# uwoseis/zephyr

Measured on AMD Instinct MI355X. Metric: wavefields/sec (freq x source solves/s) on 1024^2 grid, higher is better.
Workload: dtype f64

## Files before the change

include/helm.h:

```cpp
#ifndef HELM_H
#define HELM_H

#include <stddef.h>

#ifdef __cplusplus
extern "C" {
#endif

typedef struct helm_op helm_op;

enum { HELM_MINIZEPHYR = 0, HELM_EURUS = 1, HELM_3D = 2  };

enum {
    HELM_BICGSTAB = 0,
    HELM_CGNR = 1,
    HELM_AUTO = 2,
    HELM_MG = 3,
    HELM_DIRECT = 4
};

enum {
    HELM_OK = 0,
    HELM_ERR_ARG = -1,
    HELM_ERR_DEVICE = -2,
    HELM_ERR_STATE = -3,
    HELM_ERR_UNSUPPORTED = -4,
    HELM_ERR_PML = -5
};

enum { HELM_RHS_NODE_MAJOR = 1, HELM_OUT_NODE_MAJOR = 2, HELM_NODE_MAJOR = 3 };

typedef struct helm_solve_opts {
    int method;
    double rtol;
    int maxit;
    int check_every;
    int batch;
    int flags;
} helm_solve_opts;

typedef struct helm_solve_info {
    int iterations;
    int status;
    int restarts;
    int method;
    double relres;
} helm_solve_info;

int helm_device_count(void);
const char *helm_version(void);

helm_op *helm_create(int device, int variant, int nz, int nx, double dx, double dz,
                     int nPML, const int *freeSurf);
helm_op *helm_create3d(int device, int nz, int ny, int nx, double dx, double dy, double dz, int nPML);
void helm_destroy(helm_op *op);
const char *helm_last_error(const helm_op *op);

int helm_set_stream(helm_op *op, void *hip_stream);

int helm_set_model(helm_op *op, const double *c, const double *rho,
                   const double *theta, const double *eps, const double *delta);

int helm_assemble(helm_op *op, double freq_re, double freq_im, double tau, double ky, double cPML);

int helm_num_blocks(const helm_op *op);
long long helm_num_points(const helm_op *op);

int helm_get_diagonals(helm_op *op, double *out);

int helm_apply(helm_op *op, int block, int adjoint, const double *X, double *Y, int nrhs);
int helm_apply_device(helm_op *op, int block, int adjoint, const void *dX, void *dY, int nrhs);

int helm_solve(helm_op *op, const double *RHS, double *U, int nrhs, long long rows,
               double premul_re, double premul_im,
               const helm_solve_opts *opts, helm_solve_info *info);
int helm_solve_device(helm_op *op, const void *dRHS, void *dU, int nrhs, long long rows,
                      double premul_re, double premul_im,
                      const helm_solve_opts *opts, helm_solve_info *info);

int helm_solve_coo(helm_op *op, const long long *row, const int *col, const double *val, long long nnz, double *U, int nrhs,
                   long long rows, double premul_re, double premul_im, const helm_solve_opts *opts, helm_solve_info *info);
void *helm_host_alloc(size_t bytes);
void helm_host_free(void *p, size_t bytes);

int helm_prefactor(helm_op *op);
int helm_prefactor_n(helm_op *op, int nrhs);
int helm_prefactor_many(helm_op **ops, int n);
int helm_set_tolerance_hint(helm_op *op, double rtol);

int helm_reserve(helm_op *op, int nrhs, long long rows, int concurrent);

typedef struct helm_timing {
    double solve_ms;
    double apply_ms;
    long long apply_launches;
    double apply_bytes;
    double factor_ms;
    double gemm_ms;
    long long gemm_launches;
    double gemm_flops;
    double gemm_big_ms;
    long long gemm_big_launches;
    double gemm_big_flops;
    double gemm_bytes;
    double gemm_sol_ms;
} helm_timing;
int helm_last_timing(const helm_op *op, helm_timing *out);
int helm_set_profiling(helm_op *op, int on);

int helm_imaging_accumulate_device(helm_op *op, const void *dUF, const void *dUB, int nsrc,
                                   const void *dScaler, void *dG);

int helm_rhs_from_coo_device(helm_op *op, const void *d_row, const void *d_col, const void *d_val, long long nnz,
                             void *dR, int nrhs, long long rows);
int helm_rhs_from_coo_device_layout(helm_op *op, const void *d_row, const void *d_col, const void *d_val, long long nnz,
                                    void *dR, int nrhs, long long rows, int flags);

int helm_set_rhs_support(helm_op *op, const void *d_bits, long long rows, int nrhs);
int helm_rhs_support_from_coo(helm_op *op, const void *d_row, const void *d_col, long long nnz, void *d_bits, long long rows, int nrhs);
int helm_sample_device(helm_op *op, const void *dU, int nsrc, long long ld, const void *d_rowptr, const void *d_col,
                       const void *d_val, int nrec, void *d_out);
int helm_sample_accumulate_device(helm_op *op, const void *dU, int nsrc, long long ld, const void *d_rowptr, const void *d_col,
                                  const void *d_val, int nrec, double alpha_re, double alpha_im, double beta_re, double beta_im, void *d_out);
int helm_axpby_device(helm_op *op, double alpha_re, double alpha_im, const void *dX, double beta_re, double beta_im, void *dY, long long n);

int helm_pool_spares(int device, int spare);
int helm_trim(void);
int helm_host_trim(void);
int helm_debug_ws_slots(int device, long long bytes);
int helm_debug_plan_cache(int device);
int helm_debug_ws_selftest(int ndev, int concurrent, long long bytes);
int helm_debug_alloc_stats(int reset, long long *slow_calls, double *worst_ms);

int helm_warm(int device);
typedef struct helm_runtime_stats {
    long long dev_allocs;  double dev_alloc_bytes;  double dev_alloc_ms;
    long long host_allocs; double host_alloc_bytes; double host_alloc_ms;
    long long events_created, streams_created;
    long long first_launches; double first_launch_ms;
    long long kernels_registered, kernels_resolved; double warm_ms;
    long long dev_frees; double dev_free_ms;
    long long sync_calls; double sync_ms;
    long long slow_syncs; double worst_sync_ms;
} helm_runtime_stats;
int helm_debug_runtime_stats(int reset, helm_runtime_stats *out);
int helm_debug_stall_watch(int start, double *worst_gap_ms, long long *gaps_over_5ms);

typedef struct helm_tuning {
    int    nd_leaf;
    double nd_ws_gb;
    int    nd_sparse_rhs;
    int    nd_stable;
    double nd_stable_thr;
    double nd_stable_safety;
    int    nd_fused_leaf;
    int    nd_fused_leaf_min;
    int    nd_gjstep;
    int    nd_gjstep_min;
    int    nd_overlap;
    int    nd_xcd_map;
    int    nd_plans;
    int    nd_direct_out;
    int    nd_many;
    int    nd_leaf_idle;
    int    auto_direct;
    int    auto_mg3;
    int    prof_ext;
    int    ws_slots;
    int    pf_prio;
    int    mg3_keep;
    int    mg3_keep_levels;
    int    mg3_galerkin;
    int    mg3_depth_model;
    int    mg3_bt_f32;
    int    mg3_otf;
    int    mg3_f32;
    double mg3_omega;
    double sync_spin_ms;
    int    sync_sleep_us;
} helm_tuning;
int helm_get_tuning(helm_tuning *out);
int helm_set_tuning(const helm_tuning *t);

int helm_direct_plan(int nz, int nx, int leaf, int *out, int cap);
int helm_direct_plan_front(int nz, int nx, int leaf, int node, long long *cells, int cap);
int helm_debug_zgemm(int device, int M, int N, int K, const double *alpha, const double *A, const double *B,
                     const double *beta, double *C, int batch);
int helm_debug_inverse(int device, int n, double *A, int batch);
int helm_debug_zgemm_bench(int device, int M, int N, int K, int batch, int variant, int reps, double *ms_out);
#define HELM_ZG_TABLE 1
#define HELM_ZG_MASKS 2
#define HELM_ZG_TM64  4
int helm_debug_zgemm_choice(int M, int N, int K, int batch, int nf_div, int force_tile, int force_slab, int have_handle, int mode, int report[5]);
typedef struct helm_zgemm_ex {
    int device, M, N, K, batch;
    int lda, ldb, ldc;
    long long sa, sb, sc;
    double alpha[2], beta[2];
    const double *A; long long a_len;
    double *B; long long b_len;
    double *C; long long c_len;
    int force_tile, force_slab;
    int xcd_map;
    int ntc;
    int zr0, zr1, zc0, zc1, sk0, sk1;
    int tm64, c_is_b;
    const int *tabB, *tabCi, *tabCo; long long tab_len;
    int tab_stride, offB, offCi, offCo;
    int ldx; long long arena_rows;
    const double *Bx, *Bx2, *Cix;
    double *Cox, *Cox2;
    int k2, cj_out; double oscale[2];
    int *act;
    int report[5];
} helm_zgemm_ex;
int helm_debug_zgemm_ex(helm_zgemm_ex *p);
int helm_debug_inverse_bench(int device, int n, const double *A, int reps, int recurse_n, double *ms_out);

int helm_mg3_axis(int n, int npml, double h, double cpml, double om_re, double om_im, int level, double *x, int *lay, double *lap,
                  int *pc, double *pw, int *n_next, int *rf, double *rw);

int helm_regrid_axis(int n_in, double h_in, int n_out, double h_out, int *start, double *taps, int cap);
typedef struct helm_regrid helm_regrid;
helm_regrid *helm_regrid_create(int device, int nz_a, int nx_a, double dz_a, double dx_a, int nz_b, int nx_b, double dz_b, double dx_b,
                                double zorig, double xorig);
void helm_regrid_destroy(helm_regrid *plan);
int helm_regrid_apply_device(helm_regrid *plan, helm_op *op, int k, const void *dIn, long long in_fstride, long long in_estride, void *dOut,
                             long long out_fstride, long long out_estride, double gain_re, double gain_im, double beta, const void *dMul);
int helm_regrid_apply(helm_regrid *plan, int k, const double *in, long long in_fstride, long long in_estride, double *out, long long out_fstride,
                      long long out_estride, double gain_re, double gain_im, double beta, const double *mul);

#ifdef __cplusplus
}
#endif
#endif
```

zephyr_amd/_lib.py:

```python
import ctypes
import os
import numpy as np

_HERE = os.path.dirname(os.path.abspath(__file__))
LIB_PATH = os.path.join(_HERE, 'libhelm.so')

HELM_MINIZEPHYR, HELM_EURUS, HELM_3D = 0, 1, 2
HELM_BICGSTAB, HELM_CGNR, HELM_AUTO, HELM_MG, HELM_DIRECT = 0, 1, 2, 3, 4
HELM_RHS_NODE_MAJOR, HELM_OUT_NODE_MAJOR, HELM_NODE_MAJOR = 1, 2, 3
METHODS = {'bicgstab': HELM_BICGSTAB, 'cgnr': HELM_CGNR, 'auto': HELM_AUTO, 'mg': HELM_MG, 'direct': HELM_DIRECT}

ERRORS = {-1: 'HELM_ERR_ARG', -2: 'HELM_ERR_DEVICE', -3: 'HELM_ERR_STATE', -4: 'HELM_ERR_UNSUPPORTED', -5: 'HELM_ERR_PML'}


class HelmError(RuntimeError):
    def __init__(self, code, text):
        self.code = code
        RuntimeError.__init__(self, '%s: %s' % (ERRORS.get(code, code), text))


class SolveOpts(ctypes.Structure):
    _fields_ = [('method', ctypes.c_int), ('rtol', ctypes.c_double), ('maxit', ctypes.c_int),
                ('check_every', ctypes.c_int), ('batch', ctypes.c_int), ('flags', ctypes.c_int)]


class SolveInfo(ctypes.Structure):
    _fields_ = [('iterations', ctypes.c_int), ('status', ctypes.c_int), ('restarts', ctypes.c_int),
                ('method', ctypes.c_int), ('relres', ctypes.c_double)]


class Timing(ctypes.Structure):
    _fields_ = [('solve_ms', ctypes.c_double), ('apply_ms', ctypes.c_double),
                ('apply_launches', ctypes.c_longlong), ('apply_bytes', ctypes.c_double),
                ('factor_ms', ctypes.c_double), ('gemm_ms', ctypes.c_double),
                ('gemm_launches', ctypes.c_longlong), ('gemm_flops', ctypes.c_double),
                ('gemm_big_ms', ctypes.c_double), ('gemm_big_launches', ctypes.c_longlong), ('gemm_big_flops', ctypes.c_double),
                ('gemm_bytes', ctypes.c_double), ('gemm_sol_ms', ctypes.c_double)]


class Tuning(ctypes.Structure):
    _fields_ = [('nd_leaf', ctypes.c_int), ('nd_ws_gb', ctypes.c_double), ('nd_sparse_rhs', ctypes.c_int), ('nd_stable', ctypes.c_int),
                ('nd_stable_thr', ctypes.c_double), ('nd_stable_safety', ctypes.c_double), ('nd_fused_leaf', ctypes.c_int),
                ('nd_fused_leaf_min', ctypes.c_int), ('nd_gjstep', ctypes.c_int), ('nd_gjstep_min', ctypes.c_int), ('nd_overlap', ctypes.c_int),
                ('nd_xcd_map', ctypes.c_int), ('nd_plans', ctypes.c_int), ('nd_direct_out', ctypes.c_int), ('nd_many', ctypes.c_int), ('nd_leaf_idle', ctypes.c_int), ('auto_direct', ctypes.c_int),
                ('auto_mg3', ctypes.c_int), ('prof_ext', ctypes.c_int), ('ws_slots', ctypes.c_int), ('pf_prio', ctypes.c_int),
                ('mg3_keep', ctypes.c_int), ('mg3_keep_levels', ctypes.c_int), ('mg3_galerkin', ctypes.c_int), ('mg3_depth_model', ctypes.c_int),
                ('mg3_bt_f32', ctypes.c_int), ('mg3_otf', ctypes.c_int), ('mg3_f32', ctypes.c_int), ('mg3_omega', ctypes.c_double), ('sync_spin_ms', ctypes.c_double), ('sync_sleep_us', ctypes.c_int)]


class RuntimeStats(ctypes.Structure):
    _fields_ = [('dev_allocs', ctypes.c_longlong), ('dev_alloc_bytes', ctypes.c_double), ('dev_alloc_ms', ctypes.c_double),
                ('host_allocs', ctypes.c_longlong), ('host_alloc_bytes', ctypes.c_double), ('host_alloc_ms', ctypes.c_double),
                ('events_created', ctypes.c_longlong), ('streams_created', ctypes.c_longlong),
                ('first_launches', ctypes.c_longlong), ('first_launch_ms', ctypes.c_double),
                ('kernels_registered', ctypes.c_longlong), ('kernels_resolved', ctypes.c_longlong), ('warm_ms', ctypes.c_double),
                ('dev_frees', ctypes.c_longlong), ('dev_free_ms', ctypes.c_double),
                ('sync_calls', ctypes.c_longlong), ('sync_ms', ctypes.c_double), ('slow_syncs', ctypes.c_longlong), ('worst_sync_ms', ctypes.c_double)]


class ZgemmEx(ctypes.Structure):
    _fields_ = [('device', ctypes.c_int), ('M', ctypes.c_int), ('N', ctypes.c_int), ('K', ctypes.c_int), ('batch', ctypes.c_int),
                ('lda', ctypes.c_int), ('ldb', ctypes.c_int), ('ldc', ctypes.c_int),
                ('sa', ctypes.c_longlong), ('sb', ctypes.c_longlong), ('sc', ctypes.c_longlong),
                ('alpha', ctypes.c_double * 2), ('beta', ctypes.c_double * 2),
                ('A', ctypes.c_void_p), ('a_len', ctypes.c_longlong), ('B', ctypes.c_void_p), ('b_len', ctypes.c_longlong),
                ('C', ctypes.c_void_p), ('c_len', ctypes.c_longlong),
                ('force_tile', ctypes.c_int), ('force_slab', ctypes.c_int), ('xcd_map', ctypes.c_int), ('ntc', ctypes.c_int),
                ('zr0', ctypes.c_int), ('zr1', ctypes.c_int), ('zc0', ctypes.c_int), ('zc1', ctypes.c_int), ('sk0', ctypes.c_int), ('sk1', ctypes.c_int),
                ('tm64', ctypes.c_int), ('c_is_b', ctypes.c_int),
                ('tabB', ctypes.c_void_p), ('tabCi', ctypes.c_void_p), ('tabCo', ctypes.c_void_p), ('tab_len', ctypes.c_longlong),
                ('tab_stride', ctypes.c_int), ('offB', ctypes.c_int), ('offCi', ctypes.c_int), ('offCo', ctypes.c_int),
                ('ldx', ctypes.c_int), ('arena_rows', ctypes.c_longlong),
                ('Bx', ctypes.c_void_p), ('Bx2', ctypes.c_void_p), ('Cix', ctypes.c_void_p), ('Cox', ctypes.c_void_p), ('Cox2', ctypes.c_void_p),
                ('k2', ctypes.c_int), ('cj_out', ctypes.c_int), ('oscale', ctypes.c_double * 2),
                ('act', ctypes.c_void_p), ('report', ctypes.c_int * 5)]


_c_dp = ctypes.POINTER(ctypes.c_double)
_SIGNATURES = {
    'helm_device_count': (ctypes.c_int, []),
    'helm_version': (ctypes.c_char_p, []),
    'helm_create': (ctypes.c_void_p, [ctypes.c_int, ctypes.c_int, ctypes.c_int, ctypes.c_int, ctypes.c_double,
                                      ctypes.c_double, ctypes.c_int, ctypes.POINTER(ctypes.c_int)]),
    'helm_create3d': (ctypes.c_void_p, [ctypes.c_int, ctypes.c_int, ctypes.c_int, ctypes.c_int, ctypes.c_double,
                                        ctypes.c_double, ctypes.c_double, ctypes.c_int]),
    'helm_destroy': (None, [ctypes.c_void_p]),
    'helm_last_error': (ctypes.c_char_p, [ctypes.c_void_p]),
    'helm_set_stream': (ctypes.c_int, [ctypes.c_void_p, ctypes.c_void_p]),
    'helm_set_model': (ctypes.c_int, [ctypes.c_void_p, ctypes.c_void_p, ctypes.c_void_p, ctypes.c_void_p,
                                      ctypes.c_void_p, ctypes.c_void_p]),
    'helm_assemble': (ctypes.c_int, [ctypes.c_void_p, ctypes.c_double, ctypes.c_double, ctypes.c_double,
                                     ctypes.c_double, ctypes.c_double]),
    'helm_num_blocks': (ctypes.c_int, [ctypes.c_void_p]),
    'helm_num_points': (ctypes.c_longlong, [ctypes.c_void_p]),
    'helm_get_diagonals': (ctypes.c_int, [ctypes.c_void_p, ctypes.c_void_p]),
    'helm_apply': (ctypes.c_int, [ctypes.c_void_p, ctypes.c_int, ctypes.c_int, ctypes.c_void_p, ctypes.c_void_p, ctypes.c_int]),
    'helm_apply_device': (ctypes.c_int, [ctypes.c_void_p, ctypes.c_int, ctypes.c_int, ctypes.c_void_p, ctypes.c_void_p, ctypes.c_int]),
    'helm_solve': (ctypes.c_int, [ctypes.c_void_p, ctypes.c_void_p, ctypes.c_void_p, ctypes.c_int, ctypes.c_longlong,
                                  ctypes.c_double, ctypes.c_double, ctypes.POINTER(SolveOpts), ctypes.POINTER(SolveInfo)]),
    'helm_solve_device': (ctypes.c_int, [ctypes.c_void_p, ctypes.c_void_p, ctypes.c_void_p, ctypes.c_int, ctypes.c_longlong,
                                         ctypes.c_double, ctypes.c_double, ctypes.POINTER(SolveOpts), ctypes.POINTER(SolveInfo)]),
    'helm_solve_coo': (ctypes.c_int, [ctypes.c_void_p, ctypes.c_void_p, ctypes.c_void_p, ctypes.c_void_p, ctypes.c_longlong, ctypes.c_void_p, ctypes.c_int,
                                      ctypes.c_longlong, ctypes.c_double, ctypes.c_double, ctypes.POINTER(SolveOpts), ctypes.POINTER(SolveInfo)]),
    'helm_host_alloc': (ctypes.c_void_p, [ctypes.c_size_t]),
    'helm_host_free': (None, [ctypes.c_void_p, ctypes.c_size_t]),
    'helm_rhs_from_coo_device_layout': (ctypes.c_int, [ctypes.c_void_p, ctypes.c_void_p, ctypes.c_void_p, ctypes.c_void_p, ctypes.c_longlong,
                                                       ctypes.c_void_p, ctypes.c_int, ctypes.c_longlong, ctypes.c_int]),
    'helm_prefactor': (ctypes.c_int, [ctypes.c_void_p]),
    'helm_prefactor_n': (ctypes.c_int, [ctypes.c_void_p, ctypes.c_int]),
    'helm_prefactor_many': (ctypes.c_int, [ctypes.POINTER(ctypes.c_void_p), ctypes.c_int]),
    'helm_reserve': (ctypes.c_int, [ctypes.c_void_p, ctypes.c_int, ctypes.c_longlong, ctypes.c_int]),
    'helm_set_tolerance_hint': (ctypes.c_int, [ctypes.c_void_p, ctypes.c_double]),
    'helm_last_timing': (ctypes.c_int, [ctypes.c_void_p, ctypes.POINTER(Timing)]),
    'helm_set_profiling': (ctypes.c_int, [ctypes.c_void_p, ctypes.c_int]),
    'helm_imaging_accumulate_device': (ctypes.c_int, [ctypes.c_void_p, ctypes.c_void_p, ctypes.c_void_p, ctypes.c_int,
                                                      ctypes.c_void_p, ctypes.c_void_p]),
    'helm_get_tuning': (ctypes.c_int, [ctypes.POINTER(Tuning)]),
    'helm_set_tuning': (ctypes.c_int, [ctypes.POINTER(Tuning)]),
    'helm_pool_spares': (ctypes.c_int, [ctypes.c_int, ctypes.c_int]),
    'helm_trim': (ctypes.c_int, []),
    'helm_host_trim': (ctypes.c_int, []),
    'helm_debug_ws_slots': (ctypes.c_int, [ctypes.c_int, ctypes.c_longlong]),
    'helm_debug_plan_cache': (ctypes.c_int, [ctypes.c_int]),
    'helm_debug_ws_selftest': (ctypes.c_int, [ctypes.c_int, ctypes.c_int, ctypes.c_longlong]),
    'helm_debug_alloc_stats': (ctypes.c_int, [ctypes.c_int, ctypes.POINTER(ctypes.c_longlong), ctypes.POINTER(ctypes.c_double)]),
    'helm_warm': (ctypes.c_int, [ctypes.c_int]),
    'helm_debug_runtime_stats': (ctypes.c_int, [ctypes.c_int, ctypes.POINTER(RuntimeStats)]),
    'helm_debug_stall_watch': (ctypes.c_int, [ctypes.c_int, ctypes.POINTER(ctypes.c_double), ctypes.POINTER(ctypes.c_longlong)]),
    'helm_rhs_from_coo_device': (ctypes.c_int, [ctypes.c_void_p, ctypes.c_void_p, ctypes.c_void_p, ctypes.c_void_p, ctypes.c_longlong,
                                                ctypes.c_void_p, ctypes.c_int, ctypes.c_longlong]),
    'helm_sample_device': (ctypes.c_int, [ctypes.c_void_p, ctypes.c_void_p, ctypes.c_int, ctypes.c_longlong, ctypes.c_void_p, ctypes.c_void_p,
                                          ctypes.c_void_p, ctypes.c_int, ctypes.c_void_p]),
    'helm_sample_accumulate_device': (ctypes.c_int, [ctypes.c_void_p, ctypes.c_void_p, ctypes.c_int, ctypes.c_longlong, ctypes.c_void_p, ctypes.c_void_p,
                                                     ctypes.c_void_p, ctypes.c_int, ctypes.c_double, ctypes.c_double, ctypes.c_double, ctypes.c_double,
                                                     ctypes.c_void_p]),
    'helm_axpby_device': (ctypes.c_int, [ctypes.c_void_p, ctypes.c_double, ctypes.c_double, ctypes.c_void_p, ctypes.c_double, ctypes.c_double,
                                         ctypes.c_void_p, ctypes.c_longlong]),
    'helm_direct_plan': (ctypes.c_int, [ctypes.c_int, ctypes.c_int, ctypes.c_int, ctypes.c_void_p, ctypes.c_int]),
    'helm_direct_plan_front': (ctypes.c_int, [ctypes.c_int, ctypes.c_int, ctypes.c_int, ctypes.c_int, ctypes.c_void_p, ctypes.c_int]),
    'helm_mg3_axis': (ctypes.c_int, [ctypes.c_int, ctypes.c_int, ctypes.c_double, ctypes.c_double, ctypes.c_double, ctypes.c_double, ctypes.c_int,
                                     ctypes.c_void_p, ctypes.c_void_p, ctypes.c_void_p, ctypes.c_void_p, ctypes.c_void_p, ctypes.c_void_p, ctypes.c_void_p,
                                     ctypes.c_void_p]),
    'helm_debug_zgemm': (ctypes.c_int, [ctypes.c_int, ctypes.c_int, ctypes.c_int, ctypes.c_int, ctypes.c_void_p, ctypes.c_void_p,
                                        ctypes.c_void_p, ctypes.c_void_p, ctypes.c_void_p, ctypes.c_int]),
    'helm_debug_zgemm_choice': (ctypes.c_int, [ctypes.c_int] * 9 + [ctypes.POINTER(ctypes.c_int)]),
    'helm_debug_zgemm_ex': (ctypes.c_int, [ctypes.POINTER(ZgemmEx)]),
    'helm_debug_inverse': (ctypes.c_int, [ctypes.c_int, ctypes.c_int, ctypes.c_void_p, ctypes.c_int]),
    'helm_debug_zgemm_bench': (ctypes.c_int, [ctypes.c_int, ctypes.c_int, ctypes.c_int, ctypes.c_int, ctypes.c_int, ctypes.c_int, ctypes.c_int,
                                              ctypes.POINTER(ctypes.c_double)]),
    'helm_set_rhs_support': (ctypes.c_int, [ctypes.c_void_p, ctypes.c_void_p, ctypes.c_longlong, ctypes.c_int]),
    'helm_rhs_support_from_coo': (ctypes.c_int, [ctypes.c_void_p, ctypes.c_void_p, ctypes.c_void_p, ctypes.c_longlong, ctypes.c_void_p, ctypes.c_longlong, ctypes.c_int]),
    'helm_regrid_axis': (ctypes.c_int, [ctypes.c_int, ctypes.c_double, ctypes.c_int, ctypes.c_double, ctypes.c_void_p, ctypes.c_void_p, ctypes.c_int]),
    'helm_regrid_create': (ctypes.c_void_p, [ctypes.c_int, ctypes.c_int, ctypes.c_int, ctypes.c_double, ctypes.c_double, ctypes.c_int, ctypes.c_int,
                                             ctypes.c_double, ctypes.c_double, ctypes.c_double, ctypes.c_double]),
    'helm_regrid_destroy': (None, [ctypes.c_void_p]),
    'helm_regrid_apply_device': (ctypes.c_int, [ctypes.c_void_p, ctypes.c_void_p, ctypes.c_int, ctypes.c_void_p, ctypes.c_longlong, ctypes.c_longlong,
                                                ctypes.c_void_p, ctypes.c_longlong, ctypes.c_longlong, ctypes.c_double, ctypes.c_double, ctypes.c_double,
                                                ctypes.c_void_p]),
    'helm_regrid_apply': (ctypes.c_int, [ctypes.c_void_p, ctypes.c_int, ctypes.c_void_p, ctypes.c_longlong, ctypes.c_longlong, ctypes.c_void_p,
                                         ctypes.c_longlong, ctypes.c_longlong, ctypes.c_double, ctypes.c_double, ctypes.c_double, ctypes.c_void_p]),
    'helm_debug_inverse_bench': (ctypes.c_int, [ctypes.c_int, ctypes.c_int, ctypes.c_void_p, ctypes.c_int, ctypes.c_int, ctypes.POINTER(ctypes.c_double)]),
}

_lib = None


def exported_symbols():
    return sorted(_SIGNATURES)


def load():
    global _lib
    if _lib is None:
        if os.environ.get('HELM_NO_TORCH_PRELOAD', '0') != '1':
            try:
                import torch
            except Exception:
                pass
        if not os.path.exists(LIB_PATH):
            raise ImportError('libhelm.so not found at %s: run `python -c "import __graft_entry__ as g; g.build()"` '
                              '(hipcc --offload-arch=gfx950).  There is no CPU fallback.' % LIB_PATH)
        lib = ctypes.CDLL(LIB_PATH)
        for name, (res, args) in _SIGNATURES.items():
            fn = getattr(lib, name)
            fn.restype = res
            fn.argtypes = args
        _lib = lib
    return _lib


def tuning():
    t = Tuning()
    check(load().helm_get_tuning(ctypes.byref(t)))
    return t


def set_tuning(t=None):
    check(load().helm_set_tuning(ctypes.byref(t) if t is not None else None))


def runtime_stats(reset=False):
    st = RuntimeStats()
    check(load().helm_debug_runtime_stats(1 if reset else 0, ctypes.byref(st)))
    return {k: getattr(st, k) for k, _ in RuntimeStats._fields_}


def last_error(handle=None):
    msg = load().helm_last_error(handle)
    return msg.decode() if msg else ''


def check(rc, handle=None):
    if rc < 0:
        raise HelmError(rc, last_error(handle))
    return rc


def require_gpu():
    n = load().helm_device_count()
    if n <= 0:
        raise HelmError(-2, 'no HIP device visible (%s); libhelm has no CPU path' % last_error(None))
    return n


class _PinnedBlock(object):

    def __init__(self, nbytes):
        self.nbytes = int(nbytes)
        self.ptr = load().helm_host_alloc(self.nbytes)
        if not self.ptr:
            raise MemoryError('helm_host_alloc(%d) failed' % self.nbytes)
        self.__array_interface__ = {'shape': (self.nbytes,), 'typestr': '|u1', 'data': (self.ptr, False), 'version': 3}

    def __del__(self):
        try:
            if self.ptr:
                load().helm_host_free(self.ptr, self.nbytes)
                self.ptr = None
        except Exception:
            pass


def pinned_empty(shape, dtype=np.complex128):
    n = int(np.prod(shape)) * np.dtype(dtype).itemsize
    if n == 0:
        return np.empty(shape, dtype=dtype)
    try:
        block = _PinnedBlock(n)
    except Exception:
        return np.empty(shape, dtype=dtype)
    return np.asarray(block).view(dtype).reshape(shape)


def pinned_reserve(shape, count, dtype=np.complex128):
    held = [pinned_empty(shape, dtype) for _ in range(int(count))]
    n = len(held)
    del held
    return n


def to_device(arr, dev, dtype=None):
    import torch
    a = np.ascontiguousarray(arr, dtype=dtype)
    if a.nbytes < (64 << 10):
        return torch.from_numpy(a).to(dev)
    host = pinned_empty(a.shape, a.dtype)
    host[...] = a
    return torch.from_numpy(host).to(dev)


_TORCH_NP = {'torch.complex128': np.complex128, 'torch.complex64': np.complex64, 'torch.float64': np.float64, 'torch.float32': np.float32,
             'torch.int64': np.int64, 'torch.int32': np.int32, 'torch.uint8': np.uint8}


def from_device(t):
    import torch
    t = t.contiguous()
    if t.numel() * t.element_size() < (64 << 10):
        return t.cpu().numpy()
    host = pinned_empty(tuple(t.shape), _TORCH_NP[str(t.dtype)])
    torch.from_numpy(host).copy_(t)
    return np.array(host)


def from_device_pinned(t):
    import torch
    t = t.contiguous()
    if t.numel() * t.element_size() < (64 << 10):
        return t.cpu().numpy()
    host = pinned_empty(tuple(t.shape), _TORCH_NP[str(t.dtype)])
    torch.from_numpy(host).copy_(t)
    return host


def wait_torch_stream(dev, spin_ms=None):
    import time
    import torch
    st = torch.cuda.current_stream(dev)
    budget = (tuning().sync_spin_ms if spin_ms is None else spin_ms) * 1e-3
    t0 = time.perf_counter()
    while budget > 0 and not st.query():
        if time.perf_counter() - t0 > budget:
            break
    st.synchronize()


def ptr(arr):
    return arr.ctypes.data_as(ctypes.c_void_p) if arr is not None else None


def c128(arr):
    return np.ascontiguousarray(arr, dtype=np.complex128)


def f64(arr):
    return np.ascontiguousarray(arr, dtype=np.float64)
```

zephyr_amd/csrc/direct.hpp:

```cpp
#pragma once
#include "helm_internal.hpp"
#include <memory>

struct NdDev {
    int z0, z1, x0, x1;
    int cut, pos;
    int dof;
    int s, m;
    int ntop, nbot, nleft, nright, xlo;
    int kid[2];
    int smax, mmax;
    long long foff;
    long long finv_off, f12_off;
    long long voff;
    long long roff;
};

struct NdGroup {
    int first = 0, cnt = 0, level = 0;
    bool leaf = false;
    int smax = 0, mmax = 0;
    long long foff = 0, voff = 0;
    long long roff = 0;
    long long finv = 0, g21 = 0, f12 = 0;
};

struct NdPlan {
    int nz = 0, nx = 0, leaf = 8, nlevels = 0, dof = 1;
    std::vector<NdDev> nodes;
    std::vector<NdGroup> groups;
    long long fac_elems = 0, fregion = 0, vregion = 0, work_elems = 0, total_rows = 0;
};

struct NdPlanDev {
    NdPlan plan;
    int device = 0;
    NdDev *d_nodes = nullptr;
    int4 *d_tab = nullptr;
    int *d_cellnode = nullptr;
    ~NdPlanDev();
};

struct NdStable {
    int node = -1;
    size_t group = 0;
    int smax = 0, mmax = 0;
    cplx *lu = nullptr;
    cplx *f21 = nullptr;
    int *piv = nullptr;
    cplx *vs = nullptr; size_t vs_elems = 0;
};

#define ND_NF_MAX 4
struct NdPlanesSet { const cplx *p[ND_NF_MAX]; };
struct NdFacShared {
    int device = 0;
    cplx *d_fac = nullptr; size_t fac_bytes = 0;
    double *d_est = nullptr; size_t est_elems = 0;
    ~NdFacShared();
};
struct NdFactor {
    std::shared_ptr<NdPlanDev> pd;
    int nf = 1, kf = 0;
    std::shared_ptr<NdFacShared> shared;
    cplx *d_fac = nullptr;
    int block = 0;
    double flops = 0;
    std::vector<NdStable> stable;
    double *d_est = nullptr; size_t est_elems = 0;
    int act_nct = 0;
    unsigned char *d_qmask = nullptr; size_t qmask_elems = 0;
    int *d_act = nullptr; size_t act_elems = 0;
    int *d_leafflag = nullptr; size_t leafflag_elems = 0;
    struct FlagSlot *flag_slot = nullptr; double flag_thr = 0;
};

inline cplx *nd_fac_at(const NdFactor *f, long long off, long long slot) { return f->d_fac + (long long)f->nf * off + (long long)f->kf * slot; }
inline long long nd_fac_stride(const NdFactor *f, long long slot) { return (long long)f->nf * slot; }

__host__ __device__ inline int nd_local(const NdDev &n, int nz, int nx, int z, int x, int comp = 0) {
    (void)nz; (void)nx;
    const int d = n.dof;
    if (n.cut < 0) { if (z >= n.z0 && z < n.z1 && x >= n.x0 && x < n.x1) return ((z - n.z0) * (n.x1 - n.x0) + (x - n.x0)) * d + comp; }
    else if (n.cut == 0) { if (z == n.pos && x >= n.x0 && x < n.x1) return (x - n.x0) * d + comp; }
    else { if (x == n.pos && z >= n.z0 && z < n.z1) return (z - n.z0) * d + comp; }
    const int wrow = n.ntop ? n.ntop : n.nbot;
    if (n.ntop && z == n.z0 - 1 && x >= n.xlo && x < n.xlo + wrow) return n.s + (x - n.xlo) * d + comp;
    if (n.nbot && z == n.z1 && x >= n.xlo && x < n.xlo + wrow) return n.s + (n.ntop + (x - n.xlo)) * d + comp;
    if (n.nleft && x == n.x0 - 1 && z >= n.z0 && z < n.z1) return n.s + (n.ntop + n.nbot + (z - n.z0)) * d + comp;
    if (n.nright && x == n.x1 && z >= n.z0 && z < n.z1) return n.s + (n.ntop + n.nbot + n.nleft + (z - n.z0)) * d + comp;
    return -1;
}

__host__ __device__ inline void nd_cell(const NdDev &n, int a, int &z, int &x, int &comp) {
    const int d = n.dof;
    if (a < n.s) {
        comp = a % d; a /= d;
        if (n.cut < 0) { const int w = n.x1 - n.x0; z = n.z0 + a / w; x = n.x0 + a % w; }
        else if (n.cut == 0) { z = n.pos; x = n.x0 + a; }
        else { z = n.z0 + a; x = n.pos; }
        return;
    }
    a -= n.s;
    comp = a % d; a /= d;
    if (a < n.ntop) { z = n.z0 - 1; x = n.xlo + a; return; }
    a -= n.ntop;
    if (a < n.nbot) { z = n.z1; x = n.xlo + a; return; }
    a -= n.nbot;
    if (a < n.nleft) { z = n.z0 + a; x = n.x0 - 1; return; }
    a -= n.nleft;
    z = n.z0 + a; x = n.x1;
}
__host__ __device__ inline void nd_cell(const NdDev &n, int a, int &z, int &x) { int comp; nd_cell(n, a, z, x, comp); }

__host__ __device__ inline int nd_pos(const NdDev &n, int a) { return a < n.s ? a : n.smax + (a - n.s); }

int nd_build_plan(NdPlan &P, int nz, int nx, int leaf, int dof = 1);
long long nd_factor_ws_elems(const NdPlan &P);
int nd_get_plan(helm_op *op, int leaf, int dof, std::shared_ptr<NdPlanDev> *out);
int nd_get_plan_dims(helm_op *op, int nz, int nx, int leaf, int dof, std::shared_ptr<NdPlanDev> *out);
int nd_factor(helm_op *op, int block, NdFactor *f, cplx *ws, const cplx *planes = nullptr);
int nd_factor_enqueue(helm_op *op, int block, NdFactor *f, cplx *ws, const cplx *planes = nullptr);
int nd_factor_enqueue_many(helm_op *op, int nf, helm_op *const *ops, NdFactor *const *fs, cplx *ws);
void nd_free(NdFactor *f);
long long nd_solve_ws_elems(const NdPlan &P, int nrhs);
int nd_solve(helm_op *op, NdFactor *f, const cplx *Xin, cplx *Xout, int nrhs, cplx *ws, int conj_out = 0);
int nd_axpy_one(helm_op *op, cplx *y, const cplx *x, long long n, int conj = 0);
struct NdDirectOut { cplx *U = nullptr; cplx oscale = {1.0, 0.0}; };
int nd_solve_nm(helm_op *op, NdFactor *f, const cplx *Qt, cplx *Xt, int nrhs, cplx *arenaV, const NdDirectOut *dout = nullptr);
int nd_factor_solve_nm(helm_op *op, int block, NdFactor *f, cplx *ws_factor, const cplx *planes, const cplx *Qt, cplx *Xt, int nrhs, cplx *arenaV,
                       hipStream_t side, float *factor_ms, const NdDirectOut *dout = nullptr);
int nd_recover_x(helm_op *op, const cplx *U, cplx *Xt, long long elems, cplx oscale);
int nd_prep_transpose_norm(helm_op *op, const cplx *rhs, long long rhs_ld, long long row_off, cplx premul, const cplx *sub, cplx *Qt, long long N, int nrhs,
                           double *part, int nblk_cap, int *nblk_out);
const unsigned char *nd_rhs_mask(helm_op *op, NdFactor *f);
struct NdResidExtra {
    int qnorm = 0;
    cplx *Uout = nullptr; int ldu = 0;
    cplx oscale = {1.0, 0.0};
    const unsigned char *qmask = nullptr;
    int xin_is_u = 0;
};
int nd_resid_nm(helm_op *op, const cplx *planes, const cplx *Xin, int ldin, cplx *Q, int ldq, const int *qmap, int ncol, int store, cplx *Rout,
                double *part, int nblk_cap, int *nblk_out, const NdResidExtra *ex = nullptr);
int nd_transpose(helm_op *op, const cplx *in, long long rows, long long cols, cplx *out);
int nd_scatter_add_cols(helm_op *op, cplx *Xt, int ldq, const int *d_cols, int k, const cplx *Dp, long long N);
int nd_pack_cols(helm_op *op, const cplx *Qt, int ldq, const int *d_cols, int k, cplx *Rp, long long N);
int nd_transpose_out(helm_op *op, const cplx *Xt, long long N, int nrhs, cplx *U, int conj);

int nd_dense_gemm(helm_op *op, int M, int N, int K, cplx alpha, const cplx *A, int lda, const cplx *B, int ldb, cplx beta, cplx *C, int ldc);
int nd_dense_gemm_batched(helm_op *op, int M, int N, int K, cplx alpha, const cplx *A, int lda, long long sa, const cplx *B, int ldb, long long sb,
                          cplx beta, cplx *C, int ldc, long long sc, int batch);
int nd_dense_inverse(helm_op *op, cplx *M, int n, cplx *W);
```

zephyr_amd/csrc/nd_factor.hip:

```cpp
#include "nd_internal.hpp"
#include <map>
#include <mutex>
#include <cstring>

namespace {

__device__ __forceinline__ long long mf_off(long long off, long long slot, int nf, int kf) { return (long long)nf * off + (long long)kf * slot; }
__device__ __forceinline__ cplx *front_entry(const NdDev &n, cplx *arenaF, cplx *fac, int r, int c, int nf = 1, int kf = 0, int fac_private = 0) {
    const int nmax = n.smax + n.mmax;
    if (r < n.smax) {
        return fac + (fac_private ? n.finv_off : mf_off(n.finv_off, (long long)n.smax * nmax, nf, kf)) + (long long)r * nmax + c;
    }
    return arenaF + mf_off(n.foff, (long long)n.mmax * nmax, nf, kf) + (long long)(r - n.smax) * nmax + c;
}

__global__ __launch_bounds__(256) void k_nd_assemble(const NdDev *nodes, int first, cplx *arenaF, cplx *fac, const cplx *planes, int nz, int nx) {
    const NdDev n = nodes[first + blockIdx.y];
    const long long N = (long long)nz * nx;
    const int tot = n.s + n.m;
    for (int a = blockIdx.x * blockDim.x + threadIdx.x; a < n.smax; a += gridDim.x * blockDim.x)
        if (a >= n.s) *front_entry(n, arenaF, fac, a, a) = cmake(1.0, 0.0);
    for (int a = blockIdx.x * blockDim.x + threadIdx.x; a < tot; a += gridDim.x * blockDim.x) {
        int z, x, ca;
        nd_cell(n, a, z, x, ca);
        const int ra = nd_pos(n, a);
        const int cb0 = n.dof > 2 ? max(ca - 1, 0) : 0, cb1 = n.dof > 2 ? min(ca + 1, n.dof - 1) : n.dof - 1;
        for (int cb = cb0; cb <= cb1; ++cb) {
            const cplx *pl = n.dof > 2 ? planes + (long long)(cb - ca + 1) * 9 * N * n.dof + (long long)ca * N
                                       : planes + (long long)(n.dof == 2 ? 2 * ca + cb : 0) * 9 * N;
            const long long pstride = n.dof > 2 ? N * n.dof : N;
            #pragma unroll
            for (int k = 0; k < 9; ++k) {
                const int z2 = z + k / 3 - 1, x2 = x + k % 3 - 1;
                if (z2 < 0 || z2 >= nz || x2 < 0 || x2 >= nx) continue;
                const int b = nd_local(n, nz, nx, z2, x2, cb);
                if (b < 0 || (a >= n.s && b >= n.s)) continue;
                *front_entry(n, arenaF, fac, ra, nd_pos(n, b)) = pl[(long long)k * pstride + (long long)z * nx + x];
            }
        }
    }
}

__global__ __launch_bounds__(256) void k_nd_extend_add(const NdDev *nodes, int first, int slot, cplx *arenaF, cplx *fac, int nz, int nx, int chunk) {
    extern __shared__ int map[];
    const NdDev p = nodes[first + blockIdx.y];
    if (p.kid[slot] < 0) return;
    const NdDev c = nodes[p.kid[slot]];
    const long long total = (long long)c.m * c.m;
    if ((long long)blockIdx.x * chunk >= total) return;
    for (int a = threadIdx.x; a < c.m; a += blockDim.x) {
        int z, x, comp;
        nd_cell(c, c.s + a, z, x, comp);
        map[a] = nd_pos(p, nd_local(p, nz, nx, z, x, comp));
    }
    __syncthreads();
    const cplx *Sc = arenaF + c.foff + c.smax;
    const int ldc = c.smax + c.mmax;
    for (long long e0 = (long long)blockIdx.x * chunk; e0 < total; e0 += (long long)gridDim.x * chunk) {
        const long long e1 = e0 + chunk < total ? e0 + chunk : total;
        for (long long e = e0 + threadIdx.x; e < e1; e += blockDim.x) {
            const int a = (int)(e / c.m), b2 = (int)(e - (long long)a * c.m);
            cplx *dst = front_entry(p, arenaF, fac, map[a], map[b2]);
            *dst = cadd(*dst, Sc[(long long)a * ldc + b2]);
        }
    }
}

template <bool OVR>
__global__ __launch_bounds__(256) void k_nd_build_front(const NdDev *nodes, int first, cplx *arenaF, cplx *fac, NdPlanesSet pset, int nz, int nx, int rb,
                                                        int skip22, NdDev ovr, int nf, int kfix) {
    constexpr int use_ovr = OVR ? 1 : 0;
    extern __shared__ int2 finfo[];
    const int kf = kfix >= 0 ? kfix : (int)(blockIdx.y % nf);
    const cplx *planes = pset.p[kf];
    NdDev n;
    if (OVR) n = ovr; else n = nodes[first + (kfix >= 0 ? blockIdx.y : blockIdx.y / nf)];
    const int nmax = n.smax + n.mmax;
    const int r0 = blockIdx.x * rb;
    if (r0 >= nmax) return;
    const bool h0 = n.kid[0] >= 0, h1 = n.kid[1] >= 0;
    NdDev c0 = NdDev(), c1 = NdDev();
    if (h0) c0 = nodes[n.kid[0]];
    if (h1) c1 = nodes[n.kid[1]];
    const int tid = threadIdx.x;
    for (int r = tid; r < nmax; r += 256) {
        int a = -1;
        if (r < n.s) a = r;
        else if (r >= n.smax && r - n.smax < n.m) a = n.s + r - n.smax;
        int2 e = make_int2(-1, 0);
        if (a >= 0) {
            int z, x, comp;
            nd_cell(n, a, z, x, comp);
            int k0 = 0, k1 = 0;
            if (h0) { const int la = nd_local(c0, nz, nx, z, x, comp); if (la >= c0.s) k0 = la - c0.s + 1; }
            if (h1) { const int la = nd_local(c1, nz, nx, z, x, comp); if (la >= c1.s) k1 = la - c1.s + 1; }
            if (n.dof > 2) { e.x = z | (x << 12) | (comp << 24); e.y = k0 | (k1 << 16); }
            else { e.x = z | (x << 16); e.y = k0 | (k1 << 14) | (comp << 28); }
        }
        finfo[r] = e;
    }
    __syncthreads();
    const long long N = (long long)nz * nx;
    const int ld0 = c0.smax + c0.mmax, ld1 = c1.smax + c1.mmax;
    const cplx *S0 = h0 ? arenaF + mf_off(c0.foff, (long long)c0.mmax * ld0, nf, kf) + c0.smax : nullptr;
    const cplx *S1 = h1 ? arenaF + mf_off(c1.foff, (long long)c1.mmax * ld1, nf, kf) + c1.smax : nullptr;
    const int r1 = r0 + rb < nmax ? r0 + rb : nmax;
    const int tx = tid & 63, ty = tid >> 6;
    const bool colmode = n.dof > 2;
    auto value = [&](int r, int c, const int2 ia, const int2 ib) -> cplx {
        cplx v = cmake(0.0, 0.0);
        if (ia.x < 0 || ib.x < 0) { if (r == c && r < n.smax) v = cmake(1.0, 0.0); return v; }
        const int za = colmode ? (ia.x & 0xfff) : (ia.x & 0xffff), xa = colmode ? ((ia.x >> 12) & 0xfff) : (ia.x >> 16);
        const int ca = colmode ? ((ia.x >> 24) & 0x7f) : ((ia.y >> 28) & 1);
        const int a0 = (colmode ? (ia.y & 0xffff) : (ia.y & 0x3fff)) - 1, a1 = (colmode ? ((ia.y >> 16) & 0xffff) : ((ia.y >> 14) & 0x3fff)) - 1;
        if (r < n.smax || c < n.smax) {
            const int zb = colmode ? (ib.x & 0xfff) : (ib.x & 0xffff), xb = colmode ? ((ib.x >> 12) & 0xfff) : (ib.x >> 16);
            const int dz = zb - za, dx = xb - xa;
            if (dz >= -1 && dz <= 1 && dx >= -1 && dx <= 1) {
                if (colmode) {
                    const int dc = ((ib.x >> 24) & 0x7f) - ca;
                    if (dc >= -1 && dc <= 1) v = planes[((long long)(dc + 1) * 9 + (dz + 1) * 3 + dx + 1) * N * n.dof + (long long)ca * N + (long long)za * nx + xa];
                } else {
                    const int blk = n.dof == 2 ? 2 * ca + ((ib.y >> 28) & 1) : 0;
                    v = planes[((long long)blk * 9 + (dz + 1) * 3 + dx + 1) * N + (long long)za * nx + xa];
                }
            }
        }
        const int b0 = (colmode ? (ib.y & 0xffff) : (ib.y & 0x3fff)) - 1, b1 = (colmode ? ((ib.y >> 16) & 0xffff) : ((ib.y >> 14) & 0x3fff)) - 1;
        if (a0 >= 0 && b0 >= 0) v = cadd(v, S0[(long long)a0 * ld0 + b0]);
        if (a1 >= 0 && b1 >= 0) v = cadd(v, S1[(long long)a1 * ld1 + b1]);
        return v;
    };
    for (int r = r0 + ty; r < r1; r += 4) {
        const int2 ia = finfo[r];
        const int cend = (skip22 && r >= n.smax) ? n.smax : nmax;
        for (int c = tx; c < cend; c += 64) *front_entry(n, arenaF, fac, r, c, nf, kf, use_ovr) = value(r, c, ia, finfo[c]);
    }
}

template <int AFTER>
__global__ __launch_bounds__(256) void k_front_cond(const cplx *M0, int ld, long long stride, const NdDev *nodes, double *out, double *rows, int smax, int nf) {
    __shared__ double red[4];
    __shared__ double dsh[LUS_NMAX];
    __shared__ unsigned char lone[LUS_NMAX];
    const cplx *M = M0 + (long long)blockIdx.x * stride;
    double *w = rows + (long long)blockIdx.x * smax;
    const int n = nodes[blockIdx.x / nf].s;
    const int lane = threadIdx.x & 63, wv = threadIdx.x >> 6;
    double best = 0.0;
    for (int i = wv; i < n; i += 4) {
        double v = 0.0, off = 0.0;
        for (int j = lane; j < n; j += 64) {
            const cplx a = M[(long long)i * ld + j];
            const double m = fabs(a.x) + fabs(a.y);
            v += AFTER ? m * w[j] : m;
            if (!AFTER && j != i) off += m;
        }
        for (int o = 32; o > 0; o >>= 1) { v += __shfl_down(v, o); if (!AFTER) off += __shfl_down(off, o); }
        v = __shfl(v, 0);
        if (!AFTER && lane == 0) { dsh[i] = v; lone[i] = off == 0.0; }
        best = fmax(best, v);
    }
    if (!AFTER) {
        __syncthreads();
        double a = 0.0, any = 0.0;
        for (int i = 0; i < n; ++i) { any = fmax(any, dsh[i]); if (!lone[i]) a = fmax(a, dsh[i]); }
        if (!(a > 0.0)) a = any > 0.0 ? any : 1.0;
        for (int i = threadIdx.x; i < n; i += 256) w[i] = lone[i] ? dsh[i] / a : 1.0;
        if (threadIdx.x == 0) out[blockIdx.x] = a;
        return;
    }
    if (lane == 0) red[wv] = best;
    __syncthreads();
    if (threadIdx.x == 0) out[blockIdx.x] = fmax(fmax(red[0], red[1]), fmax(red[2], red[3]));
}
__global__ void k_front_flag(const double *a, const double *b, int cnt, double scale, double thr, int *list, int cap, int nf, int kf) {
    for (int j = blockIdx.x * blockDim.x + threadIdx.x; j < cnt; j += gridDim.x * blockDim.x)
        if (!(scale * a[(long long)j * nf + kf] * b[(long long)j * nf + kf] <= thr)) {
            const int slot = atomicAdd(list, 1);
            if (slot < cap) list[1 + slot] = j;
        }
}
__global__ __launch_bounds__(256) void k_lu_factor64(cplx *A0, int ld, int n, int *piv) {
    __shared__ cplx A[64][65];
    __shared__ double rv[256];
    __shared__ int ri[256];
    const int tid = threadIdx.x;
    for (int e = tid; e < n * n; e += 256) A[e / n][e % n] = A0[(long long)(e / n) * ld + e % n];
    __syncthreads();
    for (int k = 0; k < n; ++k) {
        double best = -1.0; int bi = k;
        for (int i = k + tid; i < n; i += 256) { const double v = cabs2(A[i][k]); if (v > best) { best = v; bi = i; } }
        rv[tid] = best; ri[tid] = bi;
        __syncthreads();
        for (int off = 32; off > 0; off >>= 1) {
            if (tid < off && (rv[tid + off] > rv[tid] || (rv[tid + off] == rv[tid] && ri[tid + off] < ri[tid]))) { rv[tid] = rv[tid + off]; ri[tid] = ri[tid + off]; }
            __syncthreads();
        }
        const int p = ri[0];
        if (tid == 0) piv[k] = p;
        if (p != k && tid < n) { const cplx t = A[k][tid]; A[k][tid] = A[p][tid]; A[p][tid] = t; }
        __syncthreads();
        const cplx d = crecip(A[k][k]);
        if (tid > k && tid < n) A[tid][k] = cmul(A[tid][k], d);
        __syncthreads();
        const int w = n - k - 1;
        for (int e = tid; e < w * w; e += 256) {
            const int i = k + 1 + e / w, j = k + 1 + e % w;
            const cplx l = A[i][k], u = A[k][j];
            cplx a = A[i][j];
            a.x = fma(-l.x, u.x, a.x); a.x = fma(l.y, u.y, a.x);
            a.y = fma(-l.x, u.y, a.y); a.y = fma(-l.y, u.x, a.y);
            A[i][j] = a;
        }
        __syncthreads();
    }
    for (int e = tid; e < n * n; e += 256) A0[(long long)(e / n) * ld + e % n] = A[e / n][e % n];
}
__global__ __launch_bounds__(256) void k_lu_factor(cplx *A, int ld, int n, int *piv) {
    __shared__ double rv[256];
    __shared__ int ri[256];
    __shared__ int psh;
    const int tid = threadIdx.x;
    for (int k = 0; k < n; ++k) {
        double best = -1.0; int bi = k;
        for (int i = k + tid; i < n; i += 256) { const double v = cabs2(A[(long long)i * ld + k]); if (v > best) { best = v; bi = i; } }
        rv[tid] = best; ri[tid] = bi;
        __syncthreads();
        for (int off = 128; off > 0; off >>= 1) {
            if (tid < off && (rv[tid + off] > rv[tid] || (rv[tid + off] == rv[tid] && ri[tid + off] < ri[tid]))) { rv[tid] = rv[tid + off]; ri[tid] = ri[tid + off]; }
            __syncthreads();
        }
        if (tid == 0) { psh = ri[0]; piv[k] = ri[0]; }
        __syncthreads();
        const int p = psh;
        if (p != k) for (int j = tid; j < n; j += 256) { const cplx t = A[(long long)k * ld + j]; A[(long long)k * ld + j] = A[(long long)p * ld + j]; A[(long long)p * ld + j] = t; }
        __syncthreads();
        const cplx d = crecip(A[(long long)k * ld + k]);
        for (int i = k + 1 + tid; i < n; i += 256) A[(long long)i * ld + k] = cmul(A[(long long)i * ld + k], d);
        __syncthreads();
        const int w = n - k - 1;
        for (int e = tid; e < w * w; e += 256) {
            const int i = k + 1 + e / w, j = k + 1 + e % w;
            const cplx l = A[(long long)i * ld + k], u = A[(long long)k * ld + j];
            cplx a = A[(long long)i * ld + j];
            a.x = fma(-l.x, u.x, a.x); a.x = fma(l.y, u.y, a.x);
            a.y = fma(-l.x, u.y, a.y); a.y = fma(-l.y, u.x, a.y);
            A[(long long)i * ld + j] = a;
        }
        __syncthreads();
    }
}
__global__ __launch_bounds__(256) void k_lu_solve(const cplx *__restrict__ LU, int ld, int n, const int *__restrict__ piv, cplx *B, int ldb, int ncols) {
    __shared__ cplx Bt[LUS_NMAX][16];
    const int tid = threadIdx.x, lane = tid & 63, wv = tid >> 6;
    const int cl = wv * 4 + (lane >> 4), p = lane & 15;
    const int j0 = blockIdx.x * 16;
    for (int e = tid; e < n * 16; e += 256) { const int i = e >> 4, c = e & 15; Bt[i][c] = j0 + c < ncols ? B[(long long)i * ldb + j0 + c] : cmake(0.0, 0.0); }
    __syncthreads();
    if (p == 0) for (int k = 0; k < n; ++k) { const int q = piv[k]; if (q != k) { const cplx t = Bt[k][cl]; Bt[k][cl] = Bt[q][cl]; Bt[q][cl] = t; } }
    __builtin_amdgcn_wave_barrier();
    constexpr int NK = LUS_NMAX / 16;
    constexpr int PD = 4;
    cplx rb[PD][NK];
    auto load_row = [&](cplx (&dst)[NK], int i, int klo, int khi) {
        #pragma unroll
        for (int q = 0; q < NK; ++q) { const int k = p + 16 * q; dst[q] = (i >= 0 && i < n && k >= klo && k < khi) ? LU[(long long)i * ld + k] : cmake(0.0, 0.0); }
    };
    #pragma unroll
    for (int u = 0; u < PD; ++u) load_row(rb[u], 1 + u, 0, 1 + u);
    for (int i0 = 1; i0 < n; i0 += PD) {
        #pragma unroll
        for (int u = 0; u < PD; ++u) {
            const int i = i0 + u;
            if (i < n) {
                cplx acc = cmake(0.0, 0.0);
                #pragma unroll
                for (int q = 0; q < NK; ++q) { const int k = p + 16 * q; if (k < i) cfma(acc, rb[u][q], Bt[k][cl]); }
                load_row(rb[u], i + PD, 0, i + PD);
                #pragma unroll
                for (int off = 8; off > 0; off >>= 1) { acc.x += __shfl_xor(acc.x, off); acc.y += __shfl_xor(acc.y, off); }
                if (p == 0) Bt[i][cl] = csub(Bt[i][cl], acc);
                __builtin_amdgcn_wave_barrier();
            }
        }
    }
    #pragma unroll
    for (int u = 0; u < PD; ++u) load_row(rb[u], n - 1 - u, n - 1 - u, n);
    for (int i0 = n - 1; i0 >= 0; i0 -= PD) {
        #pragma unroll
        for (int u = 0; u < PD; ++u) {
            const int i = i0 - u;
            if (i >= 0) {
                cplx acc = cmake(0.0, 0.0), d = cmake(1.0, 0.0);
                #pragma unroll
                for (int q = 0; q < NK; ++q) { const int k = p + 16 * q; if (k > i && k < n) cfma(acc, rb[u][q], Bt[k][cl]); if (k == i) d = rb[u][q]; }
                load_row(rb[u], i - PD, i - PD, n);
                #pragma unroll
                for (int off = 8; off > 0; off >>= 1) { acc.x += __shfl_xor(acc.x, off); acc.y += __shfl_xor(acc.y, off); }
                const int src = (lane & 48) | (i & 15);
                const double dx = __shfl(d.x, src), dy = __shfl(d.y, src);
                if (p == 0) Bt[i][cl] = cmul(csub(Bt[i][cl], acc), crecip(cmake(dx, dy)));
                __builtin_amdgcn_wave_barrier();
            }
        }
    }
    __syncthreads();
    for (int e = tid; e < n * 16; e += 256) { const int i = e >> 4, c = e & 15; if (j0 + c < ncols) B[(long long)i * ldb + j0 + c] = Bt[i][c]; }
}

}

void launch_lu_solve(hipStream_t st, const cplx *LU, int ld, int n, const int *piv, cplx *B, int ldb, int ncols) {
    HELM_LAUNCH(k_lu_solve, dim3((ncols + 15) / 16), dim3(256), 0, st, LU, ld, n, piv, B, ldb, ncols);
}

static void stable_free(NdFactor *f) {
    const int dev = f->pd ? f->pd->device : 0;
    for (NdStable &st : f->stable) {
        const size_t nmax = (size_t)st.smax + st.mmax;
        helm_pool_free(dev, st.lu, (size_t)st.smax * nmax * sizeof(cplx));
        helm_pool_free(dev, st.f21, (size_t)std::max(1, st.mmax) * st.smax * sizeof(cplx));
        helm_pool_free(dev, st.piv, (size_t)st.smax * sizeof(int));
        helm_pool_free(dev, st.vs, st.vs_elems * sizeof(cplx));
    }
    f->stable.clear();
}

struct FlagSlot { int *host = nullptr; hipEvent_t ev = nullptr; int device = 0; };
namespace { std::mutex g_flag_mu; std::map<int, std::vector<FlagSlot *>> g_flag_idle; }
FlagSlot *flag_slot_acquire(int device) {
    {
        std::lock_guard<std::mutex> lk(g_flag_mu);
        std::vector<FlagSlot *> &idle = g_flag_idle[device];
        if (!idle.empty()) { FlagSlot *s = idle.back(); idle.pop_back(); return s; }
    }
    FlagSlot *s = new FlagSlot(); s->device = device;
    s->host = (int *)helm_hostpool_alloc((ND_STABLE_CAP + 1) * sizeof(int));
    if (!s->host) { delete s; return nullptr; }
    if (hipEventCreateWithFlags(&s->ev, hipEventDisableTiming) != hipSuccess) { (void)hipGetLastError(); helm_hostpool_free(s->host, (ND_STABLE_CAP + 1) * sizeof(int)); delete s; return nullptr; }
    return s;
}
void flag_slot_release(FlagSlot *s) {
    if (!s) return;
    std::lock_guard<std::mutex> lk(g_flag_mu);
    g_flag_idle[s->device].push_back(s);
}

void nd_free(NdFactor *f) {
    if (!f) return;
    stable_free(f);
    if (f->flag_slot) { (void)hipEventSynchronize(f->flag_slot->ev); flag_slot_release(f->flag_slot); f->flag_slot = nullptr; }
    if (f->d_est && !f->shared) helm_pool_free(f->pd ? f->pd->device : 0, f->d_est, f->est_elems * sizeof(double));
    if (f->d_leafflag) helm_pool_free(f->pd ? f->pd->device : 0, f->d_leafflag, f->leafflag_elems * sizeof(int));
    if (f->d_act) helm_pool_free(f->pd ? f->pd->device : 0, f->d_act, f->act_elems * sizeof(int));
    if (f->d_qmask) helm_pool_free(f->pd ? f->pd->device : 0, f->d_qmask, f->qmask_elems);
    if (f->d_fac && !f->shared) helm_pool_free(f->pd ? f->pd->device : 0, f->d_fac, (size_t)f->pd->plan.fac_elems * sizeof(cplx));
    delete f;
}
NdFacShared::~NdFacShared() {
    if (d_fac) helm_pool_free(device, d_fac, fac_bytes);
    if (d_est) helm_pool_free(device, d_est, est_elems * sizeof(double));
}

bool merged_group(const NdPlan &P, const NdGroup &g) { (void)P; return g.mmax > 0 && g.leaf; }

namespace {

bool stable_enabled(const NdPlan &P) {
    return helm_tuning_now().nd_stable != 0 && P.dof == 1;
}
const size_t kEstList = (ND_STABLE_CAP + 2) / 2 + 2;
size_t est_list_off(const NdPlan &P, int nf) {
    int maxcnt = 1;
    for (const NdGroup &g : P.groups) maxcnt = std::max(maxcnt, g.cnt);
    return 2 * (size_t)nf * maxcnt;
}
size_t est_rows_off(const NdPlan &P, int nf) { return est_list_off(P, nf) + (size_t)nf * kEstList + 8; }
int ensure_est(helm_op *op, NdFactor *f, int stable_smax) {
    const NdPlan &P = f->pd->plan;
    const int nf = f->nf;
    size_t rows = 0;
    for (const NdGroup &g : P.groups) if (!g.leaf && g.mmax > 0 && g.smax <= stable_smax) rows = std::max(rows, (size_t)g.cnt * g.smax);
    const size_t need = est_rows_off(P, nf) + (size_t)nf * rows;
    if (f->est_elems >= need) return HELM_OK;
    if (f->shared) {
        if (f->shared->d_est) { hipStreamSynchronize(op->stream); helm_pool_free(op->device, f->shared->d_est, f->shared->est_elems * sizeof(double)); f->shared->d_est = nullptr; f->shared->est_elems = 0; }
        f->shared->d_est = (double *)helm_pool_alloc(op->device, need * sizeof(double));
        if (!f->shared->d_est) return HELM_ERR_DEVICE;
        f->shared->est_elems = need;
        f->d_est = f->shared->d_est; f->est_elems = need;
        return HELM_OK;
    }
    if (f->d_est) { hipStreamSynchronize(op->stream); helm_pool_free(op->device, f->d_est, f->est_elems * sizeof(double)); f->d_est = nullptr; f->est_elems = 0; }
    f->d_est = (double *)helm_pool_alloc(op->device, need * sizeof(double));
    if (!f->d_est) return HELM_ERR_DEVICE;
    f->est_elems = need;
    return HELM_OK;
}

int flag_group(helm_op *op, NdFactor *f, size_t gi, double *est, double rt_hint) {
    const NdPlan &P = f->pd->plan;
    const NdGroup &g = P.groups[gi];
    hipStream_t st = op->stream;
    const helm_tuning tune = helm_tuning_now();
    const double safety = tune.nd_stable_safety;
    const double rt = rt_hint > 0 ? rt_hint : 1e-10;
    const double thr = tune.nd_stable_thr > 0 ? tune.nd_stable_thr : std::min(1e9, std::max(2e3, rt / (safety * 1.1102230246251565e-16)));
    if (!f->flag_slot) f->flag_slot = flag_slot_acquire(op->device);
    FlagSlot *slot = f->flag_slot;
    if (!slot) HELM_FAIL(op, HELM_ERR_DEVICE, "direct solver: no pinned buffer for the list of ill-conditioned fronts");
    f->flag_thr = thr;
    int *d_list = (int *)(est + est_list_off(P, f->nf) + (size_t)f->kf * kEstList);
    HIP_TRY(op, hipMemsetAsync(d_list, 0, sizeof(int), st));
    HELM_LAUNCH(k_front_flag, dim3((g.cnt + 255) / 256), dim3(256), 0, st, (const double *)est, (const double *)(est + (size_t)f->nf * g.cnt), g.cnt, 1.0, thr, d_list, ND_STABLE_CAP,
                f->nf, f->kf);
    HIP_TRY(op, hipMemcpyAsync(slot->host, d_list, (ND_STABLE_CAP + 1) * sizeof(int), hipMemcpyDeviceToHost, st));
    HIP_TRY(op, hipEventRecord(slot->ev, st));
    return HELM_OK;
}

int stabilise_group(helm_op *op, NdFactor *f, size_t gi, cplx *arenaF, cplx *work, const cplx *planes, const double *est) {
    const NdPlan &P = f->pd->plan;
    const NdGroup &g = P.groups[gi];
    hipStream_t st = op->stream;
    const int nmax = g.smax + g.mmax;
    const int nf = f->nf, kf = f->kf;
    FlagSlot *slot = f->flag_slot;
    if (!slot) HELM_FAIL(op, HELM_ERR_STATE, "direct solver: stabilise_group without flag_group");
    int h_list[ND_STABLE_CAP + 1];
    {
        const hipError_t es = hipEventSynchronize(slot->ev);
        memcpy(h_list, slot->host, sizeof(h_list));
        f->flag_slot = nullptr; flag_slot_release(slot);
        if (es != hipSuccess) HELM_FAIL(op, HELM_ERR_DEVICE, "direct solver: waiting for the list of ill-conditioned fronts failed: %s", hipGetErrorString(es));
    }
    const int nflag = std::max(0, std::min(h_list[0], ND_STABLE_CAP));
    if (h_list[0] > ND_STABLE_CAP) {
        std::vector<double> eh(2 * (size_t)nf * g.cnt);
        HIP_TRY(op, hipStreamSynchronize(st));
        HIP_TRY(op, hipMemcpy(eh.data(), est, eh.size() * sizeof(double), hipMemcpyDeviceToHost));
        const double thr = f->flag_thr;
        std::vector<std::pair<double, int>> cand;
        for (int j = 0; j < g.cnt; ++j) {
            const double e = eh[(size_t)j * nf + kf] * eh[(size_t)nf * g.cnt + (size_t)j * nf + kf];
            if (!(e <= thr)) cand.push_back(std::make_pair(e == e ? e : HUGE_VAL, j));
        }
        auto worse = [](const std::pair<double, int> &a, const std::pair<double, int> &b) { return a.first != b.first ? a.first > b.first : a.second < b.second; };
        const int take = std::min<int>(nflag, (int)cand.size());
        std::partial_sort(cand.begin(), cand.begin() + take, cand.end(), worse);
        for (int q = 0; q < take; ++q) h_list[1 + q] = cand[q].second;
    }
    std::sort(h_list + 1, h_list + 1 + nflag);
    if (getenv("HELM_ND_DEBUG") && atoi(getenv("HELM_ND_DEBUG")) >= 2) {
        std::vector<double> h(2 * (size_t)nf * g.cnt);
        hipStreamSynchronize(st);
        hipMemcpy(h.data(), est, h.size() * sizeof(double), hipMemcpyDeviceToHost);
        double worst = 0; int wj = 0;
        for (int j = 0; j < g.cnt; ++j) { const double e = h[(size_t)j * nf + kf] * h[(size_t)nf * g.cnt + (size_t)j * nf + kf]; if (!(e <= worst)) { worst = e; wj = j; } }
        fprintf(stderr, "[helm direct] level %d s %d cnt %d (frequency %d of %d): estimate of front 0 = %.3e * %.3e; worst %.3e at %d; flagged %d\n", g.level, g.smax, g.cnt, kf, nf, h[kf], h[(size_t)nf * g.cnt + kf], worst, wj, h_list[0]);
    }
    if ((long long)g.smax * g.mmax > P.work_elems) return HELM_OK;
    const cplx one = cmake(1, 0), mone = cmake(-1, 0);
    for (int q = 0; q < nflag; ++q) {
        const int j = h_list[1 + q];
        NdStable S;
        S.node = g.first + j; S.group = gi; S.smax = g.smax; S.mmax = g.mmax;
        S.lu = (cplx *)helm_pool_alloc(op->device, (size_t)g.smax * nmax * sizeof(cplx));
        S.f21 = (cplx *)helm_pool_alloc(op->device, (size_t)std::max(1, g.mmax) * g.smax * sizeof(cplx));
        S.piv = (int *)helm_pool_alloc(op->device, (size_t)g.smax * sizeof(int));
        f->stable.push_back(S);
        if (!S.lu || !S.f21 || !S.piv) HELM_FAIL(op, HELM_ERR_DEVICE, "direct solver: allocation for an ill-conditioned front failed");
        NdDev n = P.nodes[S.node];
        const long long foff = (long long)nf * n.foff + (long long)kf * g.mmax * nmax;
        n.finv_off = 0; n.f12_off = g.smax;
        const int rb = std::max(std::min(nmax, 4), (nmax + 2047) / 2048);
        NdPlanesSet ps; for (int q2 = 0; q2 < ND_NF_MAX; ++q2) ps.p[q2] = planes;
        HELM_LAUNCH(k_nd_build_front<true>, dim3((nmax + rb - 1) / rb, 1), dim3(256), (size_t)nmax * sizeof(int2), st, f->pd->d_nodes, 0, arenaF, S.lu, ps, P.nz, P.nx, rb,
                           0, n, nf, kf);
        cplx *F21 = arenaF + foff, *F22 = arenaF + foff + g.smax;
        HIP_TRY(op, hipMemcpy2DAsync(S.f21, (size_t)g.smax * sizeof(cplx), F21, (size_t)nmax * sizeof(cplx), (size_t)g.smax * sizeof(cplx), (size_t)g.mmax, hipMemcpyDeviceToDevice, st));
        if (g.smax <= 64) HELM_LAUNCH(k_lu_factor64, dim3(1), dim3(256), 0, st, S.lu, nmax, g.smax, S.piv);
        else HELM_LAUNCH(k_lu_factor, dim3(1), dim3(256), 0, st, S.lu, nmax, g.smax, S.piv);
        HIP_TRY(op, hipMemcpy2DAsync(work, (size_t)g.mmax * sizeof(cplx), S.lu + g.smax, (size_t)nmax * sizeof(cplx), (size_t)g.mmax * sizeof(cplx), (size_t)g.smax, hipMemcpyDeviceToDevice, st));
        HELM_LAUNCH(k_lu_solve, dim3((g.mmax + 15) / 16), dim3(256), 0, st, (const cplx *)S.lu, nmax, g.smax, (const int *)S.piv, work, g.mmax, g.mmax);
        gemm(op, g.mmax, g.mmax, g.smax, mone, S.f21, g.smax, 0, work, g.mmax, 0, one, F22, nmax, 0, 1, nullptr);
        if (getenv("HELM_ND_DEBUG") && atoi(getenv("HELM_ND_DEBUG")) >= 3) {
            auto sum2d = [&](const void *src, size_t pitch, size_t wbytes, size_t rows_) {
                std::vector<unsigned char> h(wbytes * rows_);
                hipMemcpy2D(h.data(), wbytes, src, pitch, wbytes, rows_, hipMemcpyDeviceToHost);
                unsigned long long x = 1469598103934665603ull;
                for (unsigned char c : h) { x ^= c; x *= 1099511628211ull; }
                return x;
            };
            hipStreamSynchronize(st);
            fprintf(stderr, "[helm direct] treated front %d (level %d, s %d of %d, m %d of %d): lu %016llx f12w %016llx piv %016llx f21 %016llx work %016llx f22 %016llx\n", S.node, g.level, n.s, g.smax, n.m, g.mmax,
                    sum2d(S.lu, (size_t)nmax * sizeof(cplx), (size_t)g.smax * sizeof(cplx), g.smax), sum2d(S.lu + g.smax, (size_t)nmax * sizeof(cplx), (size_t)g.mmax * sizeof(cplx), g.smax),
                    sum2d(S.piv, (size_t)g.smax * sizeof(int), (size_t)g.smax * sizeof(int), 1),
                    sum2d(S.f21, (size_t)g.smax * sizeof(cplx), (size_t)g.smax * sizeof(cplx), g.mmax), sum2d(work, (size_t)g.mmax * sizeof(cplx), (size_t)g.mmax * sizeof(cplx), g.smax),
                    sum2d(F22, (size_t)nmax * sizeof(cplx), (size_t)g.mmax * sizeof(cplx), g.mmax));
        }
    }
    const int dbg = getenv("HELM_ND_DEBUG") ? atoi(getenv("HELM_ND_DEBUG")) : 0;
    if (dbg && nflag) fprintf(stderr, "[helm direct] level %d (%s, s = %d, m = %d): %d ill-conditioned front(s) re-eliminated with a pivoted LU\n", g.level, g.leaf ? "leaves" : "separators", g.smax, g.mmax, nflag);
    return check_kernels(op, "re-elimination of ill-conditioned fronts");
}

}

int factor_group_set(helm_op *op, const FacSet &S, size_t gi, cplx *arenaF, cplx *work) {
    NdFactor *f0 = S.f[0];
    const int nf = S.nf;
    const NdPlan &P = f0->pd->plan;
    const NdDev *d_nodes = f0->pd->d_nodes;
    hipStream_t st = op->stream;
    const cplx one = cmake(1, 0), mone = cmake(-1, 0), zero = cmake(0, 0);
    const NdGroup &g = P.groups[gi];
    const int nmax = g.smax + g.mmax;
    const long long fs = (long long)g.mmax * nmax;
    const long long s11 = (long long)g.smax * g.smax, s12 = (long long)g.smax * g.mmax, s1 = (long long)g.smax * nmax;
    const int nbatch = nf * g.cnt;
    cplx *F = arenaF + (long long)nf * g.foff;
    cplx *Finv = f0->d_fac + (long long)nf * g.finv, *G21 = f0->d_fac + (long long)nf * g.g21, *F12 = Finv + g.smax;
    NfDivScope nfdiv(nf);
    const helm_tuning tune = helm_tuning_now();
    const int fused_leaf = tune.nd_fused_leaf;
    const int fused_leaf_min = tune.nd_fused_leaf_min;
    if (fused_leaf && g.leaf && g.cnt >= fused_leaf_min && P.dof == 1 && P.leaf <= 8 && g.smax <= 64 && g.mmax > 0 && g.mmax <= LEAF_MP) {
        const int leaf_dbg = getenv("HELM_LEAF_DBG") ? atoi(getenv("HELM_LEAF_DBG")) : 0;
        for (int k = 0; k < nf; ++k) {
            NdFactor *f = S.f[k];
            if (f->leafflag_elems < (size_t)g.cnt) {
                if (f->d_leafflag) { hipStreamSynchronize(st); helm_pool_free(op->device, f->d_leafflag, f->leafflag_elems * sizeof(int)); f->d_leafflag = nullptr; f->leafflag_elems = 0; }
                int maxcnt = g.cnt;
                for (const NdGroup &q : P.groups) if (q.leaf) maxcnt = std::max(maxcnt, q.cnt);
                f->d_leafflag = (int *)helm_pool_alloc(op->device, (size_t)maxcnt * sizeof(int));
                if (!f->d_leafflag) HELM_FAIL(op, HELM_ERR_DEVICE, "direct solver: allocation of the leaf flags failed");
                f->leafflag_elems = (size_t)maxcnt;
            }
            for (int j0 = 0; j0 < g.cnt; j0 += 65535) {
                const int nb = std::min(65535, g.cnt - j0);
                cplx *g21b = G21 + (long long)j0 * nf * g.mmax * g.smax;
                launch_leaf_factor(st, g.smax, nb, d_nodes, g.first + j0, arenaF, f0->d_fac, g21b, S.planes[k], P.nz, P.nx, f->d_leafflag + j0, leaf_dbg, nf, k);
            }
            f->flops += (double)g.cnt * 8.0 * (2.0 * LEAF_BW * g.smax * (g.smax + g.mmax) + 3.0 * g.mmax * (g.smax + g.mmax));
        }
        return HELM_OK;
    }
    bool schur_gather = false;
    const bool packs = P.dof <= 2 ? (nmax < (1 << 14) && P.nz < 65536 && P.nx < 32768) : (nmax < 65535 && P.nz < 4096 && P.nx < 4096 && P.dof < 128);
    if ((size_t)nmax * sizeof(int2) <= 64 * 1024 && packs)
        schur_gather = !g.leaf && g.mmax > 0 && P.dof == 1;
    if ((size_t)nmax * sizeof(int2) <= 64 * 1024 && packs) {
        const int want = std::max(1, 2048 / g.cnt);
        const int rb = std::max(std::min(nmax, 4), (nmax + want - 1) / want);
        NdPlanesSet ps; for (int k = 0; k < ND_NF_MAX; ++k) ps.p[k] = S.planes[k < nf ? k : 0];
        const int chunk = 65535 / nf;
        for (int j0 = 0; j0 < g.cnt; j0 += chunk) {
            const int nb = std::min(chunk, g.cnt - j0);
            HELM_LAUNCH(k_nd_build_front<false>, dim3((nmax + rb - 1) / rb, nb * nf), dim3(256), (size_t)nmax * sizeof(int2), st, d_nodes, g.first + j0, arenaF, f0->d_fac, ps,
                               P.nz, P.nx, rb, schur_gather ? 1 : 0, NdDev(), nf, -1);
        }
    } else {
        if (nf != 1) HELM_FAIL(op, HELM_ERR_UNSUPPORTED, "direct solver: fronts of %d unknowns take the unfused build, which factors one frequency at a time", nmax);
        const cplx *planes = S.planes[0];
        if (fs > 0) HIP_TRY(op, hipMemsetAsync(F, 0, (size_t)g.cnt * fs * sizeof(cplx), st));
        HIP_TRY(op, hipMemsetAsync(Finv, 0, (size_t)g.cnt * s1 * sizeof(cplx), st));
        for (int j0 = 0; j0 < g.cnt; j0 += 65535) {
            const int nb = std::min(65535, g.cnt - j0);
            HELM_LAUNCH(k_nd_assemble, dim3((nmax + 255) / 256, nb), dim3(256), 0, st, d_nodes, g.first + j0, arenaF, f0->d_fac, planes, P.nz, P.nx);
        }
        if (!g.leaf) {
            const size_t shm = (size_t)(2 * nmax + 8) * sizeof(int);
            for (int slot = 0; slot < 2; ++slot)
                for (int j0 = 0; j0 < g.cnt; j0 += 65535) {
                    const int nb = std::min(65535, g.cnt - j0);
                    const long long total = (long long)nmax * nmax;
                    const int chunk = (int)std::max<long long>(4096, std::min<long long>(total, std::max<long long>(16LL * nmax, total / std::max(1, 2048 / nb))));
                    const int gx = (int)std::max<long long>(1, std::min<long long>((total + chunk - 1) / chunk, 65535));
                    HELM_LAUNCH(k_nd_extend_add, dim3(gx, nb), dim3(256), shm, st, d_nodes, g.first + j0, slot, arenaF, f0->d_fac, P.nz, P.nx, chunk);
                }
        }
    }
    const int stable_smax = 128;
    const bool watch = stable_enabled(P) && !g.leaf && g.mmax > 0 && g.smax <= std::min(stable_smax, LUS_NMAX) && ensure_est(op, f0, std::min(stable_smax, LUS_NMAX)) == HELM_OK;
    double *est = watch ? f0->d_est : nullptr;
    double *est_rows = watch ? est + est_rows_off(P, nf) : nullptr;
    if (watch) for (int b0 = 0; b0 < nbatch; b0 += 65535 / nf * nf)
        HELM_LAUNCH(k_front_cond<0>, dim3(std::min(65535 / nf * nf, nbatch - b0)), dim3(256), 0, st, Finv + (long long)b0 * s1, nmax, s1, d_nodes + g.first + b0 / nf, est + b0,
                           est_rows + (long long)b0 * g.smax, g.smax, nf);
    invert(op, Finv, nmax, s1, g.smax, nbatch, work, s11, P.dof, 0);
    if (watch) for (int b0 = 0; b0 < nbatch; b0 += 65535 / nf * nf)
        HELM_LAUNCH(k_front_cond<1>, dim3(std::min(65535 / nf * nf, nbatch - b0)), dim3(256), 0, st, Finv + (long long)b0 * s1, nmax, s1, d_nodes + g.first + b0 / nf, est + nbatch + b0,
                           est_rows + (long long)b0 * g.smax, g.smax, nf);
    if (watch) for (int k = 0; k < nf; ++k) { const int rcf = flag_group(op, S.f[k], gi, est, S.rtol[k]); if (rcf) return rcf; }
    if (g.mmax > 0) {
        gemm(op, g.mmax, g.smax, g.smax, one, F, nmax, fs, Finv, nmax, s1, zero, G21, g.smax, (long long)g.mmax * g.smax, nbatch);
        if (schur_gather) {
            GemmRows R; R.schur4 = 1; R.nodes = d_nodes; R.first = g.first; R.arenaS = arenaF; R.tabCi = f0->pd->d_tab + g.roff; R.tab_stride = nmax; R.nf = nf;
            gemm(op, g.mmax, g.mmax, g.smax, mone, G21, g.smax, (long long)g.mmax * g.smax, F12, nmax, s1, zero, F + g.smax, nmax, fs, nbatch, &R);
        } else
        gemm(op, g.mmax, g.mmax, g.smax, mone, G21, g.smax, (long long)g.mmax * g.smax, F12, nmax, s1, one, F + g.smax, nmax, fs, nbatch);
        if (merged_group(P, g)) {
            if (g.smax <= 64) {
                GemmRows R; R.dense = 1; R.tm64 = 1;
                gemm(op, g.smax, g.mmax, g.smax, mone, Finv, nmax, s1, F12, nmax, s1, zero, F12, nmax, s1, nbatch, &R);
            } else {
                gemm(op, g.smax, g.mmax, g.smax, mone, Finv, nmax, s1, F12, nmax, s1, zero, work, g.mmax, s12, nbatch);
                HIP_TRY(op, hipMemcpy2DAsync(F12, (size_t)nmax * sizeof(cplx), work, (size_t)g.mmax * sizeof(cplx), (size_t)g.mmax * sizeof(cplx),
                                             (size_t)nbatch * g.smax, hipMemcpyDeviceToDevice, st));
            }
        }
    }
    for (int k = 0; k < nf; ++k)
        S.f[k]->flops += (double)g.cnt * 8.0 * (2.0 * g.smax * g.smax * g.smax + (double)g.smax * g.smax * g.mmax + (double)g.smax * g.mmax * g.mmax);
    if (watch) for (int k = 0; k < nf; ++k) { const int rcs = stabilise_group(op, S.f[k], gi, arenaF, work, S.planes[k], est); if (rcs) return rcs; }
    return HELM_OK;
}

int factor_group(helm_op *op, NdFactor *f, size_t gi, cplx *arenaF, cplx *work, const cplx *planes) {
    FacSet S; S.nf = 1; S.f[0] = f; S.planes[0] = planes; S.rtol[0] = op->rtol_hint;
    return factor_group_set(op, S, gi, arenaF, work);
}

int factor_prologue(helm_op *op, int block, NdFactor *f, const cplx *planes_in, const cplx **planes) {
    const NdPlan &P = f->pd->plan;
    if (!f->d_fac) {
        f->d_fac = (cplx *)helm_pool_alloc(op->device, (size_t)P.fac_elems * sizeof(cplx));
        if (!f->d_fac) HELM_FAIL(op, HELM_ERR_DEVICE, "direct solver: cannot allocate %.1f GB for the factors", P.fac_elems * 16e-9);
    }
    *planes = planes_in ? planes_in : (P.dof == 2 ? op->d_C : op->d_C + (long long)block * op->nplanes * op->N);
    f->block = block; f->flops = 0;
    return HELM_OK;
}

long long nd_factor_ws_elems(const NdPlan &P) { return 2 * P.fregion + P.work_elems; }

int nd_factor(helm_op *op, int block, NdFactor *f, cplx *ws, const cplx *planes_in) {
    const NdPlan &P = f->pd->plan;
    const cplx *planes = nullptr;
    int rc = factor_prologue(op, block, f, planes_in, &planes);
    if (rc) return rc;
    GroupTrace tr(op->stream, "factor");
    for (size_t gi = 0; gi < P.groups.size(); ++gi) {
        rc = factor_group(op, f, gi, ws, ws + 2 * P.fregion, planes);
        if (rc) return rc;
        tr.mark();
    }
    tr.report(P, false);
    HIP_TRY(op, hipStreamSynchronize(op->stream));
    return check_kernels(op, "factorisation kernels");
}

int nd_factor_enqueue(helm_op *op, int block, NdFactor *f, cplx *ws, const cplx *planes_in) {
    const NdPlan &P = f->pd->plan;
    const cplx *planes = nullptr;
    int rc = factor_prologue(op, block, f, planes_in, &planes);
    if (rc) return rc;
    GroupTrace tr(op->stream, "factor");
    for (size_t gi = 0; gi < P.groups.size(); ++gi) {
        rc = factor_group(op, f, gi, ws, ws + 2 * P.fregion, planes);
        if (rc) return rc;
        tr.mark();
    }
    tr.report(P, false);
    return check_kernels(op, "factorisation kernels");
}

int nd_factor_enqueue_many(helm_op *op, int nf, helm_op *const *ops, NdFactor *const *fs, cplx *ws) {
    if (nf < 1 || nf > ND_NF_MAX) HELM_FAIL(op, HELM_ERR_ARG, "direct solver: %d frequencies in one factorisation (1 .. %d)", nf, ND_NF_MAX);
    const NdPlan &P = fs[0]->pd->plan;
    if (P.dof != 1) HELM_FAIL(op, HELM_ERR_UNSUPPORTED, "direct solver: the coupled system is factored one frequency at a time");
    std::shared_ptr<NdFacShared> sh = std::make_shared<NdFacShared>();
    sh->device = op->device;
    sh->fac_bytes = (size_t)nf * (size_t)P.fac_elems * sizeof(cplx);
    sh->d_fac = (cplx *)helm_pool_alloc(op->device, sh->fac_bytes);
    if (!sh->d_fac) HELM_FAIL(op, HELM_ERR_DEVICE, "direct solver: cannot allocate %.1f GB for the factors of %d frequencies", sh->fac_bytes * 1e-9, nf);
    FacSet S; S.nf = nf;
    for (int k = 0; k < nf; ++k) {
        NdFactor *f = fs[k];
        if (f->pd.get() != fs[0]->pd.get()) HELM_FAIL(op, HELM_ERR_ARG, "direct solver: the operators of one factorisation must share their grid");
        f->nf = nf; f->kf = k; f->shared = sh; f->d_fac = sh->d_fac; f->block = 0; f->flops = 0;
        S.f[k] = f; S.planes[k] = ops[k]->d_C; S.rtol[k] = ops[k]->rtol_hint;
    }
    cplx *arenaF = ws, *work = ws + (long long)nf * 2 * P.fregion;
    GroupTrace tr(op->stream, nf == 2 ? "factor x2" : (nf == 3 ? "factor x3" : "factor x4"));
    for (size_t gi = 0; gi < P.groups.size(); ++gi) {
        const int rc = factor_group_set(op, S, gi, arenaF, work);
        if (rc) return rc;
        tr.mark();
    }
    tr.report(P, false);
    for (int k = 1; k < nf; ++k) { fs[k]->d_est = nullptr; fs[k]->est_elems = 0; }
    return check_kernels(op, "factorisation kernels");
}
```

zephyr_amd/csrc/nd_internal.hpp:

```cpp
#pragma once
#include "helm_internal.hpp"
#include "direct.hpp"
#include <hip/hip_ext.h>
#include <algorithm>

struct GjPivotArgs { const cplx *T0; int ld; long long stride; int n, k0, nb; const cplx *Wc0, *Wr0; long long wstride; cplx *Pb0; long long pstride; int batch; };
struct GemmRows {
    const int4 *tabB = nullptr, *tabCi = nullptr, *tabCo = nullptr;
    int offB = 0, offCi = 0, offCo = 0, tab_stride = 0;
    const cplx *Bx = nullptr, *Cix = nullptr; cplx *Cox = nullptr;
    int ldx = 0;
    int z0 = 0;
    int fwd3 = 0;
    int zr0 = 0, zr1 = 0, zc0 = 0, zc1 = 0;
    int sk0 = 0, sk1 = 0;
    int ksplit = 0, kc = 0; long long pstride = 0;
    int dense = 0;
    const cplx *Bx2 = nullptr; int k2 = 0;
    int tm64 = 0;
    const GjPivotArgs *la = nullptr;
    int schur4 = 0;
    const NdDev *nodes = nullptr; int first = 0;
    const cplx *arenaS = nullptr;
    int nf = 1;
    int *act = nullptr; int nct = 0;
    const int *list = nullptr, *lcount = nullptr;
    const int *act_ro = nullptr;
    int idle_done = 0;
    int hint = 0;
    int ntc = 0;
    int xcd_map = 0;
    int child_rows = 0;
    int cj_out = 0; cplx oscale = {1.0, 0.0}; cplx *Cox2 = nullptr;
};
#define GB_KIDX 512

#define PNB 32
#define LEAF_BW 9
#define LEAF_MP 36
#define LUS_NMAX 128
#define ND_STABLE_CAP 32

extern thread_local hipEvent_t tl_ev0, tl_ev1;
extern thread_local int tl_nf_div;
struct NfDivScope { int prev; explicit NfDivScope(int nf) : prev(tl_nf_div) { tl_nf_div = nf < 1 ? 1 : nf; } ~NfDivScope() { tl_nf_div = prev; } };
#define ZG_LAUNCH(KERNEL, GRID, ...) do { HelmFirstLaunch fl_(HelmKernelReg<(KERNEL)>::slot); \
                                          if (tl_ev0) hipExtLaunchKernelGGL(KERNEL, GRID, dim3(256), 0, st, tl_ev0, tl_ev1, 0, __VA_ARGS__); \
                                          else hipLaunchKernelGGL(KERNEL, GRID, dim3(256), 0, st, __VA_ARGS__); } while (0)

inline double gemm_operand_bytes(int M, int Nn, int K, cplx beta, const GemmRows *rows = nullptr) {
    const bool rd = !(beta.x == 0.0 && beta.y == 0.0);
    if (rows && rows->fwd3) return 16.0 * ((double)M * K + (double)K * Nn + (double)rows->child_rows * Nn + (double)M * Nn + (double)K * Nn);
    if (rows && rows->schur4) return 16.0 * ((double)M * K + (double)K * Nn + 1.5 * (double)M * Nn);
    return 16.0 * ((double)M * K + (double)K * Nn + (double)M * Nn * (rd ? 2.0 : 1.0));
}
inline double gemm_sol_ms(double flops, double bytes) { return 1e3 * std::max(flops / 78.6e12, bytes / 8.0e12); }

struct ExtArm {
    helm_op *op; bool on; double fl, by; long long shape[5];
    ExtArm(helm_op *o, bool e, double f, double b, int m_, int n_, int k_, int nb_, int mode_) : op(o), on(false), fl(f), by(b), shape{m_, n_, k_, nb_, mode_} {
        if (!e) return;
        if (op->ev_used + 2 > op->ev_pool.size() && op->ev_pool.size() < 16384) (void)helm_events_grow(op, 64);
        if (op->ev_used + 2 <= op->ev_pool.size()) { tl_ev0 = op->ev_pool[op->ev_used]; tl_ev1 = op->ev_pool[op->ev_used + 1]; on = true; }
    }
    ~ExtArm() {
        if (!on) return;
        op->ev_pending_gemm.push_back(std::make_pair((int)op->ev_used, fl));
        op->ev_pending_gemm_n.push_back(1);
        op->ev_pending_gemm_bytes.push_back(by);
        op->ev_pending_gemm_sol.push_back(gemm_sol_ms(fl, by));
        for (int q = 0; q < 5; ++q) op->ev_pending_gemm_shape.push_back(shape[q]);
        op->ev_used += 2;
        tl_ev0 = tl_ev1 = nullptr;
    }
};

struct GemmRun {
    helm_op *op;
    explicit GemmRun(helm_op *o) : op(o) { if (op && op->gemm_run_depth++ == 0) { op->gemm_run_pair = -1; op->gemm_run_flops = 0; op->gemm_run_bytes = 0; op->gemm_run_sol = 0; op->gemm_run_launches = 0; } }
    ~GemmRun() {
        if (!op || --op->gemm_run_depth != 0) return;
        if (op->gemm_run_pair >= 0 && op->gemm_run_launches > 0) {
            hipEventRecord(op->ev_pool[op->gemm_run_pair + 1], op->stream);
            op->ev_pending_gemm.push_back(std::make_pair(op->gemm_run_pair, op->gemm_run_flops));
            op->ev_pending_gemm_n.push_back(op->gemm_run_launches);
            op->ev_pending_gemm_bytes.push_back(op->gemm_run_bytes);
            op->ev_pending_gemm_sol.push_back(op->gemm_run_sol);
        }
        op->gemm_run_pair = -1;
    }
};

typedef double v4f64 __attribute__((ext_vector_type(4)));
typedef double v2f64 __attribute__((ext_vector_type(2)));

#define GJ_MAX 64
template <int NMAX>
__device__ __forceinline__ void gj_lds(cplx (*a)[NMAX + 1], cplx *fcol, int *piv, int n, int tid, int nthreads) {
    for (int k = 0; k < n; ++k) {
        if (tid < 64) {
            double val = (tid >= k && tid < n) ? cabs2(a[tid][k]) : -1.0;
            int idx = tid;
            for (int off = 32; off > 0; off >>= 1) {
                const double ov = __shfl_down(val, off);
                const int oi = __shfl_down(idx, off);
                if (ov > val) { val = ov; idx = oi; }
            }
            const int p = __shfl(idx, 0);
            if (tid == 0) piv[k] = p;
            if (tid < n) {
                const cplx f = (tid == p) ? a[k][k] : a[tid][k];
                const cplx rk = a[p][tid], rp = a[k][tid];
                const cplx d = crecip(a[p][k]);
                a[p][tid] = rp;
                a[k][tid] = (tid == k) ? d : cmul(rk, d);
                fcol[tid] = f;
            }
        }
        __syncthreads();
        for (int e = tid; e < n * n; e += nthreads) {
            const int i = e / n, j = e % n;
            if (i == k) continue;
            cplx base = (j == k) ? cmake(0.0, 0.0) : a[i][j];
            a[i][j] = csub(base, cmul(fcol[i], a[k][j]));
        }
        __syncthreads();
    }
    if (tid < 64) {
        for (int k = n - 1; k >= 0; --k) {
            const int p = piv[k];
            if (p != k && tid < n) { cplx t = a[tid][k]; a[tid][k] = a[tid][p]; a[tid][p] = t; }
        }
    }
    __syncthreads();
}

inline int check_kernels(helm_op *op, const char *what) {
    hipError_t e = hipGetLastError();
    if (e != hipSuccess) { char b[256]; snprintf(b, sizeof(b), "direct solver: %s failed: %s", what, hipGetErrorString(e)); helm_set_error(op, b); return HELM_ERR_DEVICE; }
    return HELM_OK;
}

struct GroupTrace {
    bool on; hipStream_t st; std::vector<hipEvent_t> ev; const char *what;
    GroupTrace(hipStream_t s, const char *w) : st(s), what(w) { const int t = getenv("HELM_ND_TRACE") ? atoi(getenv("HELM_ND_TRACE")) : 0; on = t != 0; mark(); }
    void mark() { if (!on) return; hipEvent_t e; hipEventCreate(&e); hipEventRecord(e, st); ev.push_back(e); }
    void report(const NdPlan &P, bool reverse) {
        if (!on) return;
        hipStreamSynchronize(st);
        double tot = 0;
        for (size_t i = 0; i + 1 < ev.size(); ++i) {
            float ms = 0.f; hipEventElapsedTime(&ms, ev[i], ev[i + 1]); tot += ms;
            const size_t gi = reverse ? P.groups.size() - 1 - i : i;
            if (gi < P.groups.size()) {
                const NdGroup &g = P.groups[gi];
                fprintf(stderr, "[nd trace] %-8s level %2d %s cnt %6d s %5d m %5d : %8.3f ms\n", what, g.level, g.leaf ? "leaf" : "sep ", g.cnt, g.smax, g.mmax, ms);
            } else fprintf(stderr, "[nd trace] %-8s extra : %8.3f ms\n", what, ms);
        }
        fprintf(stderr, "[nd trace] %-8s total %8.3f ms\n", what, tot);
        for (hipEvent_t e : ev) hipEventDestroy(e);
        ev.clear();
    }
};

struct GemmChoice { int tile = 0, kslab = 8, xr = 0, ksplit = 0, kc = 0; };
int gemm(helm_op *op, int M, int Nn, int K, cplx alpha, const cplx *A, int lda, long long sa, const cplx *B, int ldb, long long sb,
         cplx beta, cplx *C, int ldc, long long sc, int batch, const GemmRows *rows = nullptr, GemmChoice *made = nullptr);
extern int g_gemm_tile;
extern int g_gemm_slab;
extern int g_gemm_xcd;
bool gemm_sep_bwd_small(helm_op *op, int smax, int mmax, int nrhs, const cplx *Finv, const cplx *F12, int lda, long long sa, int batch, const GemmRows &rows);
void invert(helm_op *op, cplx *M, int ld, long long stride, int n, int batch, cplx *W, long long ws, int align = 1, int base = 0);
extern int g_recurse_min;
void launch_zgemm3_la(hipStream_t st, bool latency_tile, int nb, int M, int Nn, int K, cplx alpha, const cplx *A, int lda, long long sa, const cplx *B, int ldb, long long sb,
                      cplx beta, cplx *C, int ldc, long long sc, const GemmRows &R, const GjPivotArgs &pv);
void launch_leaf_factor(hipStream_t st, int smax, int nb, const NdDev *d_nodes, int first, cplx *arenaF, cplx *fac, cplx *g21b, const cplx *planes, int nz, int nx, int *flags, int dbg,
                        int nf = 1, int kf = 0);
struct FacSet { int nf = 1; NdFactor *f[ND_NF_MAX] = {nullptr, nullptr, nullptr, nullptr}; const cplx *planes[ND_NF_MAX] = {nullptr, nullptr, nullptr, nullptr}; double rtol[ND_NF_MAX] = {0, 0, 0, 0}; };
int factor_prologue(helm_op *op, int block, NdFactor *f, const cplx *planes_in, const cplx **planes);
int factor_group(helm_op *op, NdFactor *f, size_t gi, cplx *arenaF, cplx *work, const cplx *planes);
bool merged_group(const NdPlan &P, const NdGroup &g);
void launch_lu_solve(hipStream_t st, const cplx *LU, int ld, int n, const int *piv, cplx *B, int ldb, int ncols);
void launch_transpose(hipStream_t st, const cplx *in, long long rows, long long cols, cplx *out, int swap, int conj);
```

zephyr_amd/csrc/nd_plan.hip:

```cpp
#include "nd_internal.hpp"
#include <mutex>
#include <map>

namespace {

struct Build {
    int nz, nx, leaf, dof;
    std::vector<NdDev> nodes;
    std::vector<int> level;
    std::vector<int> parent;
};

void fill_geometry(NdDev &n, int nz, int nx, int dof) {
    const int h = n.z1 - n.z0, w = n.x1 - n.x0;
    n.dof = dof;
    n.s = dof * (n.cut < 0 ? h * w : (n.cut == 0 ? w : h));
    n.xlo = std::max(n.x0 - 1, 0);
    const int xhi = std::min(n.x1, nx - 1);
    const int wrow = xhi - n.xlo + 1;
    n.ntop = n.z0 > 0 ? wrow : 0;
    n.nbot = n.z1 < nz ? wrow : 0;
    n.nleft = n.x0 > 0 ? h : 0;
    n.nright = n.x1 < nx ? h : 0;
    n.m = dof * (n.ntop + n.nbot + n.nleft + n.nright);
}

int build_rec(Build &B, int z0, int z1, int x0, int x1, int lev, int parent) {
    NdDev n = NdDev();
    n.z0 = z0; n.z1 = z1; n.x0 = x0; n.x1 = x1; n.kid[0] = n.kid[1] = -1;
    const int h = z1 - z0, w = x1 - x0;
    const int me = (int)B.nodes.size();
    if (h <= B.leaf && w <= B.leaf) { n.cut = -1; n.pos = -1; }
    else if (h >= w) { n.cut = 0; n.pos = z0 + h / 2; }
    else { n.cut = 1; n.pos = x0 + w / 2; }
    fill_geometry(n, B.nz, B.nx, B.dof);
    B.nodes.push_back(n); B.level.push_back(lev); B.parent.push_back(parent);
    if (n.cut == 0) {
        int k = 0;
        if (n.pos > z0) { int c = build_rec(B, z0, n.pos, x0, x1, lev + 1, me); B.nodes[me].kid[k++] = c; }
        if (z1 > n.pos + 1) { int c = build_rec(B, n.pos + 1, z1, x0, x1, lev + 1, me); B.nodes[me].kid[k++] = c; }
    } else if (n.cut == 1) {
        int k = 0;
        if (n.pos > x0) { int c = build_rec(B, z0, z1, x0, n.pos, lev + 1, me); B.nodes[me].kid[k++] = c; }
        if (x1 > n.pos + 1) { int c = build_rec(B, z0, z1, n.pos + 1, x1, lev + 1, me); B.nodes[me].kid[k++] = c; }
    }
    return me;
}

}

int nd_build_plan(NdPlan &P, int nz, int nx, int leaf, int dof) {
    Build B; B.nz = nz; B.nx = nx; B.leaf = std::max(2, leaf); B.dof = dof;
    build_rec(B, 0, nz, 0, nx, 0, -1);
    const int nn = (int)B.nodes.size();
    int maxlev = 0;
    for (int l : B.level) maxlev = std::max(maxlev, l);
    std::vector<int> order; order.reserve(nn);
    P.groups.clear();
    for (int lev = maxlev; lev >= 0; --lev) {
        int smode = 0;
        {
            std::vector<int> hist;
            for (int i = 0; i < nn; ++i)
                if (B.level[i] == lev && B.nodes[i].cut < 0) { if ((int)hist.size() <= B.nodes[i].s) hist.resize(B.nodes[i].s + 1, 0); hist[B.nodes[i].s] += 1; }
            for (int v = 0; v < (int)hist.size(); ++v) if (hist[v] > (smode < (int)hist.size() ? hist[smode] : 0)) smode = v;
        }
        for (int kind = 0; kind < 3; ++kind) {
            NdGroup g = NdGroup(); g.first = (int)order.size(); g.level = lev; g.leaf = kind < 2;
            for (int i = 0; i < nn; ++i) {
                if (B.level[i] != lev) continue;
                const bool isleaf = B.nodes[i].cut < 0;
                const int k = !isleaf ? 2 : (B.nodes[i].s <= smode ? 0 : 1);
                if (k != kind) continue;
                order.push_back(i);
                g.smax = std::max(g.smax, B.nodes[i].s); g.mmax = std::max(g.mmax, B.nodes[i].m);
            }
            g.cnt = (int)order.size() - g.first;
            if (g.cnt > 0) P.groups.push_back(g);
        }
    }
    std::vector<int> newidx(nn);
    for (int k = 0; k < nn; ++k) newidx[order[k]] = k;
    P.nodes.resize(nn);
    for (int k = 0; k < nn; ++k) {
        NdDev n = B.nodes[order[k]];
        for (int c = 0; c < 2; ++c) if (n.kid[c] >= 0) n.kid[c] = newidx[n.kid[c]];
        P.nodes[k] = n;
    }
    P.nz = nz; P.nx = nx; P.leaf = B.leaf; P.nlevels = maxlev + 1; P.total_rows = 0; P.dof = dof;
    std::vector<long long> lev_f(maxlev + 1, 0), lev_v(maxlev + 1, 0);
    long long fac = 0;
    for (size_t gi = 0; gi < P.groups.size(); ++gi) {
        NdGroup &g = P.groups[gi];
        const long long nmax = g.smax + g.mmax;
        g.foff = lev_f[g.level]; g.voff = lev_v[g.level];
        g.roff = P.total_rows; P.total_rows += (long long)g.cnt * nmax;
        lev_f[g.level] += (long long)g.cnt * g.mmax * nmax;
        lev_v[g.level] += (long long)g.cnt * nmax;
        g.finv = fac; g.f12 = fac + g.smax; fac += (long long)g.cnt * g.smax * nmax;
        g.g21 = fac; fac += (long long)g.cnt * g.mmax * g.smax;
    }
    P.fac_elems = fac;
    P.fregion = 0; P.vregion = 0; P.work_elems = 0;
    for (int l = 0; l <= maxlev; ++l) { P.fregion = std::max(P.fregion, lev_f[l]); P.vregion = std::max(P.vregion, lev_v[l]); }
    for (size_t gi = 0; gi < P.groups.size(); ++gi) {
        NdGroup &g = P.groups[gi];
        g.foff += (long long)(g.level & 1) * P.fregion;
        g.voff += (long long)(g.level & 1) * P.vregion;
        P.work_elems = std::max(P.work_elems, (long long)g.cnt * g.smax * (g.leaf ? std::max(g.smax, g.mmax) : g.smax));
        for (int j = 0; j < g.cnt; ++j) {
            NdDev &n = P.nodes[g.first + j];
            const long long nmax = g.smax + g.mmax;
            n.smax = g.smax; n.mmax = g.mmax;
            n.foff = g.foff + (long long)j * g.mmax * nmax;
            n.finv_off = g.finv + (long long)j * g.smax * nmax;
            n.f12_off = n.finv_off + g.smax;
            n.voff = g.voff + (long long)j * nmax;
            n.roff = g.roff + (long long)j * nmax;
        }
    }
    return HELM_OK;
}
namespace {

__global__ __launch_bounds__(256) void k_nd_cellnode(const int4 *tab, long long rows, int nmax, int first, int *cellnode) {
    for (long long r = (long long)blockIdx.x * blockDim.x + threadIdx.x; r < rows; r += (long long)gridDim.x * blockDim.x) {
        const int4 e = tab[r];
        if (e.w && e.x >= 0) cellnode[e.x] = first + (int)(r / nmax);
    }
}

__global__ __launch_bounds__(256) void k_nd_build_tab(const NdDev *nodes, int first, int4 *tab, int nz, int nx) {
    const NdDev n = nodes[first + blockIdx.y];
    const int nmax = n.smax + n.mmax;
    for (int row = blockIdx.x * blockDim.x + threadIdx.x; row < nmax; row += gridDim.x * blockDim.x) {
        int a = -1;
        if (row < n.s) a = row;
        else if (row >= n.smax && row - n.smax < n.m) a = n.s + row - n.smax;
        int4 e = make_int4(-1, -1, -1, row < n.s ? 1 : 0);
        if (a >= 0) {
            int z, x, comp;
            nd_cell(n, a, z, x, comp);
            e.x = comp * nz * nx + z * nx + x;
            for (int k = 0; k < 2; ++k) {
                if (n.kid[k] < 0) continue;
                const NdDev c = nodes[n.kid[k]];
                const int la = nd_local(c, nz, nx, z, x, comp);
                if (la >= c.s) { const int src = (int)(c.voff + c.smax + (la - c.s)); if (k == 0) e.y = src; else e.z = src; }
            }
        }
        tab[n.roff + row] = e;
    }
}

}

NdPlanDev::~NdPlanDev() {
    if (d_nodes) helm_pool_free(device, d_nodes, plan.nodes.size() * sizeof(NdDev));
    if (d_tab) helm_pool_free(device, d_tab, (size_t)plan.total_rows * sizeof(int4));
    if (d_cellnode) helm_pool_free(device, d_cellnode, (size_t)plan.nz * plan.nx * sizeof(int));
}

namespace {
std::mutex g_plan_mu;
std::map<int, std::vector<std::shared_ptr<NdPlanDev>>> &g_plans = *new std::map<int, std::vector<std::shared_ptr<NdPlanDev>>>();

std::shared_ptr<NdPlanDev> plan_lookup(int device, int pnz, int pnx, int leaf, int dof) {
    std::vector<std::shared_ptr<NdPlanDev>> &L = g_plans[device];
    for (size_t i = 0; i < L.size(); ++i) {
        const NdPlanDev &c = *L[i];
        if (c.plan.nz == pnz && c.plan.nx == pnx && c.plan.leaf == std::max(2, leaf) && c.plan.dof == dof) {
            std::shared_ptr<NdPlanDev> hit = L[i];
            L.erase(L.begin() + i); L.push_back(hit);
            return hit;
        }
    }
    return nullptr;
}
}

int nd_get_plan(helm_op *op, int leaf, int dof, std::shared_ptr<NdPlanDev> *out) { return nd_get_plan_dims(op, op->nz, op->nx, leaf, dof, out); }

int nd_get_plan_dims(helm_op *op, int pnz, int pnx, int leaf, int dof, std::shared_ptr<NdPlanDev> *out) {
    {
        std::lock_guard<std::mutex> lk(g_plan_mu);
        if (std::shared_ptr<NdPlanDev> hit = plan_lookup(op->device, pnz, pnx, leaf, dof)) { *out = hit; return HELM_OK; }
    }
    std::shared_ptr<NdPlanDev> pd(new NdPlanDev());
    pd->device = op->device;
    nd_build_plan(pd->plan, pnz, pnx, leaf, dof);
    const NdPlan &P = pd->plan;
    if (2 * P.vregion >= (1LL << 31) || P.total_rows >= (1LL << 31)) HELM_FAIL(op, HELM_ERR_UNSUPPORTED, "direct solver: grid too large for 32-bit row indices");
    pd->d_nodes = (NdDev *)helm_pool_alloc(op->device, P.nodes.size() * sizeof(NdDev));
    pd->d_tab = (int4 *)helm_pool_alloc(op->device, (size_t)P.total_rows * sizeof(int4));
    if (!pd->d_nodes || !pd->d_tab) HELM_FAIL(op, HELM_ERR_DEVICE, "direct solver: allocation of the plan tables failed");
    HIP_TRY(op, hipMemcpyAsync(pd->d_nodes, P.nodes.data(), P.nodes.size() * sizeof(NdDev), hipMemcpyHostToDevice, op->stream));
    for (size_t gi = 0; gi < P.groups.size(); ++gi) {
        const NdGroup &g = P.groups[gi];
        const int nmax = g.smax + g.mmax;
        for (int j0 = 0; j0 < g.cnt; j0 += 65535) {
            const int nb = std::min(65535, g.cnt - j0);
            HELM_LAUNCH(k_nd_build_tab, dim3((nmax + 255) / 256, nb), dim3(256), 0, op->stream, pd->d_nodes, g.first + j0, pd->d_tab, P.nz, P.nx);
        }
    }
    if (dof == 1) {
        pd->d_cellnode = (int *)helm_pool_alloc(op->device, (size_t)pnz * pnx * sizeof(int));
        if (pd->d_cellnode) {
            HIP_TRY(op, hipMemsetAsync(pd->d_cellnode, 0xFF, (size_t)pnz * pnx * sizeof(int), op->stream));
            for (size_t gi = 0; gi < P.groups.size(); ++gi) {
                const NdGroup &g = P.groups[gi];
                if (!g.leaf) continue;
                const long long rows = (long long)g.cnt * (g.smax + g.mmax);
                HELM_LAUNCH(k_nd_cellnode, dim3((unsigned)std::min<long long>((rows + 255) / 256, 65535)), dim3(256), 0, op->stream,
                                   (const int4 *)(pd->d_tab + g.roff), rows, g.smax + g.mmax, g.first, pd->d_cellnode);
            }
        }
    }
    HIP_TRY(op, hipStreamSynchronize(op->stream));
    const int keep = helm_tuning_now().nd_plans;
    std::shared_ptr<NdPlanDev> evicted;
    {
        std::lock_guard<std::mutex> lk(g_plan_mu);
        if (std::shared_ptr<NdPlanDev> hit = plan_lookup(op->device, pnz, pnx, leaf, dof)) { *out = hit; return HELM_OK; }
        std::vector<std::shared_ptr<NdPlanDev>> &L = g_plans[op->device];
        L.push_back(pd);
        if ((int)L.size() > keep) { evicted = L.front(); L.erase(L.begin()); }
    }
    *out = pd;
    return HELM_OK;
}

extern "C" int helm_debug_plan_cache(int device) {
    helm_tuning_refresh();
    std::lock_guard<std::mutex> lk(g_plan_mu);
    auto it = g_plans.find(device);
    return it == g_plans.end() ? 0 : (int)it->second.size();
}

extern "C" int helm_direct_plan(int nz, int nx, int leaf, int *out, int cap) {
    helm_tuning_refresh();
    NdPlan P;
    nd_build_plan(P, nz, nx, leaf);
    const int nn = (int)P.nodes.size();
    if (!out) return nn;
    for (int i = 0; i < nn && i < cap; ++i) {
        const NdDev &n = P.nodes[i];
        int *o = out + 12 * i;
        o[0] = n.z0; o[1] = n.z1; o[2] = n.x0; o[3] = n.x1; o[4] = n.cut; o[5] = n.pos; o[6] = n.s; o[7] = n.m;
        o[8] = n.kid[0]; o[9] = n.kid[1]; o[10] = n.smax; o[11] = n.mmax;
    }
    return nn;
}

extern "C" int helm_direct_plan_front(int nz, int nx, int leaf, int node, long long *cells, int cap) {
    helm_tuning_refresh();
    NdPlan P;
    nd_build_plan(P, nz, nx, leaf);
    if (node < 0 || node >= (int)P.nodes.size()) return HELM_ERR_ARG;
    const NdDev &n = P.nodes[node];
    for (int a = 0; a < n.s + n.m; ++a) {
        int z, x;
        nd_cell(n, a, z, x);
        if (z < 0 || z >= nz || x < 0 || x >= nx) return -100;
        if (nd_local(n, nz, nx, z, x) != a) return -101;
        if (cells && a < cap) cells[a] = (long long)z * nx + x;
    }
    return n.s + n.m;
}
```

Before: 15910.

## Precompute front assembly table at plan time and flatten build-front work distribution

Moves the per-row assembly metadata (cell coordinates and child Schur indices) out of every front-build launch into a plan-time device table that is cached with the plan. The build-front kernel now walks a flat element range split across blocks by a balancing rule, processes two entries per thread to overlap gathers, and loads the table into LDS, or reads it from L2 when an environment switch is set. The aim is to avoid recomputing nd_cell/nd_local on each factorization and to even out block load. The cost is extra plan memory, plus new debug entry points for checking the table and kernel output.

```diff
diff --git a/include/helm.h b/include/helm.h
--- a/include/helm.h
+++ b/include/helm.h
@@ -216,6 +216,19 @@
 } helm_zgemm_ex;
 int helm_debug_zgemm_ex(helm_zgemm_ex *p);
 int helm_debug_inverse_bench(int device, int n, const double *A, int reps, int recurse_n, double *ms_out);
+int helm_debug_plan_nodes(int nz, int nx, int leaf, int dof, long long *out, int cap);
+long long helm_debug_asm_table(int device, int nz, int nx, int leaf, int dof, int *out, long long cap_rows);
+typedef struct helm_front_build {
+    int device, nz, nx, leaf, dof, group;
+    int mode, nf, skip22, front, kf;
+    int freq_id[4];
+    unsigned long long seed;
+    const double *planes[4]; long long planes_len;
+    double *image; long long image_len;
+    long long stray;
+    unsigned long long sentinel;
+} helm_front_build;
+int helm_debug_front_build(helm_front_build *p);
 
 int helm_mg3_axis(int n, int npml, double h, double cpml, double om_re, double om_im, int level, double *x, int *lay, double *lap,
                   int *pc, double *pw, int *n_next, int *rf, double *rw);
diff --git a/zephyr_amd/_lib.py b/zephyr_amd/_lib.py
--- a/zephyr_amd/_lib.py
+++ b/zephyr_amd/_lib.py
@@ -160,7 +160,19 @@
     'helm_regrid_apply': (ctypes.c_int, [ctypes.c_void_p, ctypes.c_int, ctypes.c_void_p, ctypes.c_longlong, ctypes.c_longlong, ctypes.c_void_p,
                                          ctypes.c_longlong, ctypes.c_longlong, ctypes.c_double, ctypes.c_double, ctypes.c_double, ctypes.c_void_p]),
     'helm_debug_inverse_bench': (ctypes.c_int, [ctypes.c_int, ctypes.c_int, ctypes.c_void_p, ctypes.c_int, ctypes.c_int, ctypes.POINTER(ctypes.c_double)]),
+    'helm_debug_plan_nodes': (ctypes.c_int, [ctypes.c_int, ctypes.c_int, ctypes.c_int, ctypes.c_int, ctypes.c_void_p, ctypes.c_int]),
+    'helm_debug_asm_table': (ctypes.c_longlong, [ctypes.c_int, ctypes.c_int, ctypes.c_int, ctypes.c_int, ctypes.c_int, ctypes.c_void_p, ctypes.c_longlong]),
+    'helm_debug_front_build': (ctypes.c_int, [ctypes.c_void_p]),
 }
+
+
+class FrontBuild(ctypes.Structure):
+    _fields_ = [('device', ctypes.c_int), ('nz', ctypes.c_int), ('nx', ctypes.c_int), ('leaf', ctypes.c_int), ('dof', ctypes.c_int), ('group', ctypes.c_int),
+                ('mode', ctypes.c_int), ('nf', ctypes.c_int), ('skip22', ctypes.c_int), ('front', ctypes.c_int), ('kf', ctypes.c_int),
+                ('freq_id', ctypes.c_int * 4), ('seed', ctypes.c_ulonglong),
+                ('planes', ctypes.c_void_p * 4), ('planes_len', ctypes.c_longlong),
+                ('image', ctypes.c_void_p), ('image_len', ctypes.c_longlong), ('stray', ctypes.c_longlong), ('sentinel', ctypes.c_ulonglong)]
+
 
 _lib = None
 
diff --git a/zephyr_amd/csrc/direct.hpp b/zephyr_amd/csrc/direct.hpp
--- a/zephyr_amd/csrc/direct.hpp
+++ b/zephyr_amd/csrc/direct.hpp
@@ -37,6 +37,7 @@
     int device = 0;
     NdDev *d_nodes = nullptr;
     int4 *d_tab = nullptr;
+    int2 *d_asm = nullptr;
     int *d_cellnode = nullptr;
     ~NdPlanDev();
 };
@@ -115,6 +116,25 @@
 
 __host__ __device__ inline int nd_pos(const NdDev &n, int a) { return a < n.s ? a : n.smax + (a - n.s); }
 
+__host__ __device__ inline bool nd_asm_packs(int dof, int nz, int nx, int nmax) {
+    return dof <= 2 ? (nmax < (1 << 14) && nz < 65536 && nx < 32768) : (nmax < 65535 && nz < 4096 && nx < 4096 && dof < 128);
+}
+__host__ __device__ inline int2 nd_asm_entry(const NdDev &n, const NdDev *c0, const NdDev *c1, int nz, int nx, int r) {
+    int2 e; e.x = -1; e.y = 0;
+    int a = -1;
+    if (r < n.s) a = r;
+    else if (r >= n.smax && r - n.smax < n.m) a = n.s + r - n.smax;
+    if (a < 0) return e;
+    int z, x, comp;
+    nd_cell(n, a, z, x, comp);
+    int k0 = 0, k1 = 0;
+    if (c0) { const int la = nd_local(*c0, nz, nx, z, x, comp); if (la >= c0->s) k0 = la - c0->s + 1; }
+    if (c1) { const int la = nd_local(*c1, nz, nx, z, x, comp); if (la >= c1->s) k1 = la - c1->s + 1; }
+    if (n.dof > 2) { e.x = z | (x << 12) | (comp << 24); e.y = k0 | (k1 << 16); }
+    else { e.x = z | (x << 16); e.y = k0 | (k1 << 14) | (comp << 28); }
+    return e;
+}
+
 int nd_build_plan(NdPlan &P, int nz, int nx, int leaf, int dof = 1);
 long long nd_factor_ws_elems(const NdPlan &P);
 int nd_get_plan(helm_op *op, int leaf, int dof, std::shared_ptr<NdPlanDev> *out);
diff --git a/zephyr_amd/csrc/nd_factor.hip b/zephyr_amd/csrc/nd_factor.hip
--- a/zephyr_amd/csrc/nd_factor.hip
+++ b/zephyr_amd/csrc/nd_factor.hip
@@ -66,8 +66,9 @@
     }
 }
 
-template <bool OVR>
-__global__ __launch_bounds__(256) void k_nd_build_front(const NdDev *nodes, int first, cplx *arenaF, cplx *fac, NdPlanesSet pset, int nz, int nx, int rb,
+#define BF_NE 2
+template <bool OVR, bool TLDS>
+__global__ __launch_bounds__(256) void k_nd_build_front(const NdDev *nodes, int first, cplx *arenaF, cplx *fac, NdPlanesSet pset, int nz, int nx, const int2 *asmtab, int share,
                                                         int skip22, NdDev ovr, int nf, int kfix) {
     constexpr int use_ovr = OVR ? 1 : 0;
     extern __shared__ int2 finfo[];
@@ -76,66 +77,138 @@
     NdDev n;
     if (OVR) n = ovr; else n = nodes[first + (kfix >= 0 ? blockIdx.y : blockIdx.y / nf)];
     const int nmax = n.smax + n.mmax;
-    const int r0 = blockIdx.x * rb;
-    if (r0 >= nmax) return;
+    const int cB = skip22 ? n.smax : nmax;
+    const int EA = n.smax * nmax, E = EA + n.mmax * cB;
+    const int e0 = blockIdx.x * share;
+    if (e0 >= E) return;
+    const int e1 = e0 + share < E ? e0 + share : E;
     const bool h0 = n.kid[0] >= 0, h1 = n.kid[1] >= 0;
     NdDev c0 = NdDev(), c1 = NdDev();
     if (h0) c0 = nodes[n.kid[0]];
     if (h1) c1 = nodes[n.kid[1]];
     const int tid = threadIdx.x;
-    for (int r = tid; r < nmax; r += 256) {
-        int a = -1;
-        if (r < n.s) a = r;
-        else if (r >= n.smax && r - n.smax < n.m) a = n.s + r - n.smax;
-        int2 e = make_int2(-1, 0);
-        if (a >= 0) {
-            int z, x, comp;
-            nd_cell(n, a, z, x, comp);
-            int k0 = 0, k1 = 0;
-            if (h0) { const int la = nd_local(c0, nz, nx, z, x, comp); if (la >= c0.s) k0 = la - c0.s + 1; }
-            if (h1) { const int la = nd_local(c1, nz, nx, z, x, comp); if (la >= c1.s) k1 = la - c1.s + 1; }
-            if (n.dof > 2) { e.x = z | (x << 12) | (comp << 24); e.y = k0 | (k1 << 16); }
-            else { e.x = z | (x << 16); e.y = k0 | (k1 << 14) | (comp << 28); }
-        }
-        finfo[r] = e;
-    }
-    __syncthreads();
+    const int2 *T = TLDS ? finfo : asmtab + n.roff;
+    if (TLDS) {
+        for (int r = tid; r < nmax; r += 256) finfo[r] = asmtab[n.roff + r];
+        __syncthreads();
+    }
     const long long N = (long long)nz * nx;
     const int ld0 = c0.smax + c0.mmax, ld1 = c1.smax + c1.mmax;
     const cplx *S0 = h0 ? arenaF + mf_off(c0.foff, (long long)c0.mmax * ld0, nf, kf) + c0.smax : nullptr;
     const cplx *S1 = h1 ? arenaF + mf_off(c1.foff, (long long)c1.mmax * ld1, nf, kf) + c1.smax : nullptr;
-    const int r1 = r0 + rb < nmax ? r0 + rb : nmax;
-    const int tx = tid & 63, ty = tid >> 6;
     const bool colmode = n.dof > 2;
-    auto value = [&](int r, int c, const int2 ia, const int2 ib) -> cplx {
-        cplx v = cmake(0.0, 0.0);
-        if (ia.x < 0 || ib.x < 0) { if (r == c && r < n.smax) v = cmake(1.0, 0.0); return v; }
-        const int za = colmode ? (ia.x & 0xfff) : (ia.x & 0xffff), xa = colmode ? ((ia.x >> 12) & 0xfff) : (ia.x >> 16);
-        const int ca = colmode ? ((ia.x >> 24) & 0x7f) : ((ia.y >> 28) & 1);
-        const int a0 = (colmode ? (ia.y & 0xffff) : (ia.y & 0x3fff)) - 1, a1 = (colmode ? ((ia.y >> 16) & 0xffff) : ((ia.y >> 14) & 0x3fff)) - 1;
-        if (r < n.smax || c < n.smax) {
-            const int zb = colmode ? (ib.x & 0xfff) : (ib.x & 0xffff), xb = colmode ? ((ib.x >> 12) & 0xfff) : (ib.x >> 16);
-            const int dz = zb - za, dx = xb - xa;
-            if (dz >= -1 && dz <= 1 && dx >= -1 && dx <= 1) {
-                if (colmode) {
-                    const int dc = ((ib.x >> 24) & 0x7f) - ca;
-                    if (dc >= -1 && dc <= 1) v = planes[((long long)(dc + 1) * 9 + (dz + 1) * 3 + dx + 1) * N * n.dof + (long long)ca * N + (long long)za * nx + xa];
-                } else {
-                    const int blk = n.dof == 2 ? 2 * ca + ((ib.y >> 28) & 1) : 0;
-                    v = planes[((long long)blk * 9 + (dz + 1) * 3 + dx + 1) * N + (long long)za * nx + xa];
+    const int smax = n.smax, dof = n.dof;
+    auto run = [&](cplx *dst, int rbase, int W, int lo, int hi) {
+        if (lo >= hi) return;
+        int idx = lo + tid;
+        int r = idx / W, c = idx - r * W;
+        const int dr = 256 / W, dc = 256 - dr * W;
+        r += rbase;
+        for (; idx < hi; idx += 256 * BF_NE) {
+            int rr[BF_NE], cc[BF_NE];
+            bool live[BF_NE], k0[BF_NE], k1[BF_NE], pad[BF_NE];
+            cplx v[BF_NE], s0[BF_NE], s1[BF_NE];
+            #pragma unroll
+            for (int u = 0; u < BF_NE; ++u) {
+                rr[u] = r; cc[u] = c; live[u] = idx + 256 * u < hi;
+                r += dr; c += dc;
+                if (c >= W) { c -= W; r += 1; }
+            }
+            #pragma unroll
+            for (int u = 0; u < BF_NE; ++u) {
+                int2 ia = make_int2(-1, 0), ib = make_int2(-1, 0);
+                if (live[u]) { ia = T[rr[u]]; ib = T[cc[u]]; }
+                v[u] = s0[u] = s1[u] = cmake(0.0, 0.0);
+                pad[u] = ia.x < 0 || ib.x < 0;
+                k0[u] = k1[u] = false;
+                if (pad[u]) continue;
+                const int za = colmode ? (ia.x & 0xfff) : (ia.x & 0xffff), xa = colmode ? ((ia.x >> 12) & 0xfff) : (ia.x >> 16);
+                const int ca = colmode ? ((ia.x >> 24) & 0x7f) : ((ia.y >> 28) & 1);
+                const int a0 = (colmode ? (ia.y & 0xffff) : (ia.y & 0x3fff)) - 1, a1 = (colmode ? ((ia.y >> 16) & 0xffff) : ((ia.y >> 14) & 0x3fff)) - 1;
+                const int b0 = (colmode ? (ib.y & 0xffff) : (ib.y & 0x3fff)) - 1, b1 = (colmode ? ((ib.y >> 16) & 0xffff) : ((ib.y >> 14) & 0x3fff)) - 1;
+                if (rr[u] < smax || cc[u] < smax) {
+                    const int zb = colmode ? (ib.x & 0xfff) : (ib.x & 0xffff), xb = colmode ? ((ib.x >> 12) & 0xfff) : (ib.x >> 16);
+                    const int dz = zb - za, dx = xb - xa;
+                    if (dz >= -1 && dz <= 1 && dx >= -1 && dx <= 1) {
+                        if (colmode) {
+                            const int dc2 = ((ib.x >> 24) & 0x7f) - ca;
+                            if (dc2 >= -1 && dc2 <= 1) v[u] = planes[((long long)(dc2 + 1) * 9 + (dz + 1) * 3 + dx + 1) * N * dof + (long long)ca * N + (long long)za * nx + xa];
+                        } else {
+                            const int blk = dof == 2 ? 2 * ca + ((ib.y >> 28) & 1) : 0;
+                            v[u] = planes[((long long)blk * 9 + (dz + 1) * 3 + dx + 1) * N + (long long)za * nx + xa];
+                        }
+                    }
                 }
-            }
-        }
-        const int b0 = (colmode ? (ib.y & 0xffff) : (ib.y & 0x3fff)) - 1, b1 = (colmode ? ((ib.y >> 16) & 0xffff) : ((ib.y >> 14) & 0x3fff)) - 1;
-        if (a0 >= 0 && b0 >= 0) v = cadd(v, S0[(long long)a0 * ld0 + b0]);
-        if (a1 >= 0 && b1 >= 0) v = cadd(v, S1[(long long)a1 * ld1 + b1]);
-        return v;
+                k0[u] = a0 >= 0 && b0 >= 0; k1[u] = a1 >= 0 && b1 >= 0;
+                if (k0[u]) s0[u] = S0[(long long)a0 * ld0 + b0];
+                if (k1[u]) s1[u] = S1[(long long)a1 * ld1 + b1];
+            }
+            #pragma unroll
+            for (int u = 0; u < BF_NE; ++u) {
+                if (!live[u]) continue;
+                cplx w = v[u];
+                if (pad[u]) { if (rr[u] == cc[u] && rr[u] < smax) w = cmake(1.0, 0.0); }
+                else {
+                    if (k0[u]) w = cadd(w, s0[u]);
+                    if (k1[u]) w = cadd(w, s1[u]);
+                }
+                dst[(long long)(rr[u] - rbase) * nmax + cc[u]] = w;
+            }
+        }
     };
-    for (int r = r0 + ty; r < r1; r += 4) {
-        const int2 ia = finfo[r];
-        const int cend = (skip22 && r >= n.smax) ? n.smax : nmax;
-        for (int c = tx; c < cend; c += 64) *front_entry(n, arenaF, fac, r, c, nf, kf, use_ovr) = value(r, c, ia, finfo[c]);
-    }
+    run(front_entry(n, arenaF, fac, 0, 0, nf, kf, use_ovr), 0, nmax, e0, e1 < EA ? e1 : EA);
+    if (n.mmax > 0 && cB > 0) run(front_entry(n, arenaF, fac, smax, 0, nf, kf, use_ovr), smax, cB, e0 > EA ? e0 - EA : 0, e1 - EA);
+}
+
+long long build_front_entries(int smax, int mmax, int skip22) { return (long long)smax * (smax + mmax) + (long long)mmax * (skip22 ? smax : smax + mmax); }
+void build_front_deal(long long E, int nbatch, int *gx, int *share) {
+    const long long by_size = std::max<long long>(1, (E + 1023) / 1024), by_fill = std::max(1, (4096 + nbatch - 1) / std::max(1, nbatch));
+    const long long g = std::min(by_size, by_fill);
+    *share = (int)((E + g - 1) / g);
+    *gx = (int)((E + *share - 1) / *share);
+}
+bool build_front_l2() { const char *e = getenv("HELM_ASM_L2"); return e && atoi(e) != 0; }
+void launch_build_front(hipStream_t st, const NdPlanDev *pd, const NdGroup &g, int j0, int nb, cplx *arenaF, cplx *fac, const NdPlanesSet &ps, int skip22, int nf) {
+    const NdPlan &P = pd->plan;
+    const int nmax = g.smax + g.mmax;
+    int gx, share;
+    build_front_deal(build_front_entries(g.smax, g.mmax, skip22), g.cnt * nf, &gx, &share);
+    if (build_front_l2())
+        HELM_LAUNCH((k_nd_build_front<false, false>), dim3(gx, nb * nf), dim3(256), 0, st, pd->d_nodes, g.first + j0, arenaF, fac, ps, P.nz, P.nx, (const int2 *)pd->d_asm, share, skip22, NdDev(), nf, -1);
+    else
+        HELM_LAUNCH((k_nd_build_front<false, true>), dim3(gx, nb * nf), dim3(256), (size_t)nmax * sizeof(int2), st, pd->d_nodes, g.first + j0, arenaF, fac, ps, P.nz, P.nx, (const int2 *)pd->d_asm, share, skip22, NdDev(), nf, -1);
+}
+void launch_build_front_one(hipStream_t st, const NdPlanDev *pd, const NdDev &n, cplx *arenaF, cplx *lu, const cplx *planes, int nf, int kf) {
+    const NdPlan &P = pd->plan;
+    const int nmax = n.smax + n.mmax;
+    int gx, share;
+    build_front_deal(build_front_entries(n.smax, n.mmax, 0), 1, &gx, &share);
+    NdPlanesSet ps; for (int q = 0; q < ND_NF_MAX; ++q) ps.p[q] = planes;
+    HELM_LAUNCH((k_nd_build_front<true, true>), dim3(gx, 1), dim3(256), (size_t)nmax * sizeof(int2), st, pd->d_nodes, 0, arenaF, lu, ps, P.nz, P.nx, (const int2 *)pd->d_asm, share,
+                       0, n, nf, kf);
+}
+int launch_build_scatter(helm_op *op, hipStream_t st, const NdPlanDev *pd, const NdGroup &g, cplx *arenaF, cplx *fac, const cplx *planes) {
+    const NdPlan &P = pd->plan;
+    const int nmax = g.smax + g.mmax;
+    const long long fs = (long long)g.mmax * nmax, s1 = (long long)g.smax * nmax;
+    if (fs > 0) HIP_TRY(op, hipMemsetAsync(arenaF + g.foff, 0, (size_t)g.cnt * fs * sizeof(cplx), st));
+    HIP_TRY(op, hipMemsetAsync(fac + g.finv, 0, (size_t)g.cnt * s1 * sizeof(cplx), st));
+    for (int j0 = 0; j0 < g.cnt; j0 += 65535) {
+        const int nb = std::min(65535, g.cnt - j0);
+        HELM_LAUNCH(k_nd_assemble, dim3((nmax + 255) / 256, nb), dim3(256), 0, st, pd->d_nodes, g.first + j0, arenaF, fac, planes, P.nz, P.nx);
+    }
+    if (!g.leaf) {
+        const size_t shm = (size_t)(2 * nmax + 8) * sizeof(int);
+        for (int slot = 0; slot < 2; ++slot)
+            for (int j0 = 0; j0 < g.cnt; j0 += 65535) {
+                const int nb = std::min(65535, g.cnt - j0);
+                const long long total = (long long)nmax * nmax;
+                const int chunk = (int)std::max<long long>(4096, std::min<long long>(total, std::max<long long>(16LL * nmax, total / std::max(1, 2048 / nb))));
+                const int gx = (int)std::max<long long>(1, std::min<long long>((total + chunk - 1) / chunk, 65535));
+                HELM_LAUNCH(k_nd_extend_add, dim3(gx, nb), dim3(256), shm, st, pd->d_nodes, g.first + j0, slot, arenaF, fac, P.nz, P.nx, chunk);
+            }
+    }
+    return HELM_OK;
 }
 
 template <int AFTER>
@@ -474,10 +547,7 @@
         NdDev n = P.nodes[S.node];
         const long long foff = (long long)nf * n.foff + (long long)kf * g.mmax * nmax;
         n.finv_off = 0; n.f12_off = g.smax;
-        const int rb = std::max(std::min(nmax, 4), (nmax + 2047) / 2048);
-        NdPlanesSet ps; for (int q2 = 0; q2 < ND_NF_MAX; ++q2) ps.p[q2] = planes;
-        HELM_LAUNCH(k_nd_build_front<true>, dim3((nmax + rb - 1) / rb, 1), dim3(256), (size_t)nmax * sizeof(int2), st, f->pd->d_nodes, 0, arenaF, S.lu, ps, P.nz, P.nx, rb,
-                           0, n, nf, kf);
+        launch_build_front_one(st, f->pd.get(), n, arenaF, S.lu, planes, nf, kf);
         cplx *F21 = arenaF + foff, *F22 = arenaF + foff + g.smax;
         HIP_TRY(op, hipMemcpy2DAsync(S.f21, (size_t)g.smax * sizeof(cplx), F21, (size_t)nmax * sizeof(cplx), (size_t)g.smax * sizeof(cplx), (size_t)g.mmax, hipMemcpyDeviceToDevice, st));
         if (g.smax <= 64) HELM_LAUNCH(k_lu_factor64, dim3(1), dim3(256), 0, st, S.lu, nmax, g.smax, S.piv);
@@ -548,39 +618,17 @@
         return HELM_OK;
     }
     bool schur_gather = false;
-    const bool packs = P.dof <= 2 ? (nmax < (1 << 14) && P.nz < 65536 && P.nx < 32768) : (nmax < 65535 && P.nz < 4096 && P.nx < 4096 && P.dof < 128);
-    if ((size_t)nmax * sizeof(int2) <= 64 * 1024 && packs)
+    const bool gather_build = (size_t)nmax * sizeof(int2) <= 64 * 1024 && nd_asm_packs(P.dof, P.nz, P.nx, nmax);
+    if (gather_build) {
         schur_gather = !g.leaf && g.mmax > 0 && P.dof == 1;
-    if ((size_t)nmax * sizeof(int2) <= 64 * 1024 && packs) {
-        const int want = std::max(1, 2048 / g.cnt);
-        const int rb = std::max(std::min(nmax, 4), (nmax + want - 1) / want);
         NdPlanesSet ps; for (int k = 0; k < ND_NF_MAX; ++k) ps.p[k] = S.planes[k < nf ? k : 0];
         const int chunk = 65535 / nf;
-        for (int j0 = 0; j0 < g.cnt; j0 += chunk) {
-            const int nb = std::min(chunk, g.cnt - j0);
-            HELM_LAUNCH(k_nd_build_front<false>, dim3((nmax + rb - 1) / rb, nb * nf), dim3(256), (size_t)nmax * sizeof(int2), st, d_nodes, g.first + j0, arenaF, f0->d_fac, ps,
-                               P.nz, P.nx, rb, schur_gather ? 1 : 0, NdDev(), nf, -1);
-        }
+        for (int j0 = 0; j0 < g.cnt; j0 += chunk)
+            launch_build_front(st, f0->pd.get(), g, j0, std::min(chunk, g.cnt - j0), arenaF, f0->d_fac, ps, schur_gather ? 1 : 0, nf);
     } else {
         if (nf != 1) HELM_FAIL(op, HELM_ERR_UNSUPPORTED, "direct solver: fronts of %d unknowns take the unfused build, which factors one frequency at a time", nmax);
-        const cplx *planes = S.planes[0];
-        if (fs > 0) HIP_TRY(op, hipMemsetAsync(F, 0, (size_t)g.cnt * fs * sizeof(cplx), st));
-        HIP_TRY(op, hipMemsetAsync(Finv, 0, (size_t)g.cnt * s1 * sizeof(cplx), st));
-        for (int j0 = 0; j0 < g.cnt; j0 += 65535) {
-            const int nb = std::min(65535, g.cnt - j0);
-            HELM_LAUNCH(k_nd_assemble, dim3((nmax + 255) / 256, nb), dim3(256), 0, st, d_nodes, g.first + j0, arenaF, f0->d_fac, planes, P.nz, P.nx);
-        }
-        if (!g.leaf) {
-            const size_t shm = (size_t)(2 * nmax + 8) * sizeof(int);
-            for (int slot = 0; slot < 2; ++slot)
-                for (int j0 = 0; j0 < g.cnt; j0 += 65535) {
-                    const int nb = std::min(65535, g.cnt - j0);
-                    const long long total = (long long)nmax * nmax;
-                    const int chunk = (int)std::max<long long>(4096, std::min<long long>(total, std::max<long long>(16LL * nmax, total / std::max(1, 2048 / nb))));
-                    const int gx = (int)std::max<long long>(1, std::min<long long>((total + chunk - 1) / chunk, 65535));
-                    HELM_LAUNCH(k_nd_extend_add, dim3(gx, nb), dim3(256), shm, st, d_nodes, g.first + j0, slot, arenaF, f0->d_fac, P.nz, P.nx, chunk);
-                }
-        }
+        const int rcb = launch_build_scatter(op, st, f0->pd.get(), g, arenaF, f0->d_fac, S.planes[0]);
+        if (rcb) return rcb;
     }
     const int stable_smax = 128;
     const bool watch = stable_enabled(P) && !g.leaf && g.mmax > 0 && g.smax <= std::min(stable_smax, LUS_NMAX) && ensure_est(op, f0, std::min(stable_smax, LUS_NMAX)) == HELM_OK;
@@ -694,3 +742,101 @@
     for (int k = 1; k < nf; ++k) { fs[k]->d_est = nullptr; fs[k]->est_elems = 0; }
     return check_kernels(op, "factorisation kernels");
 }
+
+namespace {
+const unsigned long long BF_SENTINEL = 0x7ff8dead5a5a5a5aull;
+inline double bf_seed_value(unsigned long long seed, int freq, long long i, int part) {
+    unsigned long long x = seed + 0x9e3779b97f4a7c15ull * (unsigned long long)(2 * i + part + 1) + 0xbf58476d1ce4e5b9ull * (unsigned long long)(freq + 1);
+    x ^= x >> 30; x *= 0xbf58476d1ce4e5b9ull; x ^= x >> 27; x *= 0x94d049bb133111ebull; x ^= x >> 31;
+    return (double)(long long)(x >> 11) / 4503599627370496.0 - 1.0;
+}
+}
+
+extern "C" int helm_debug_front_build(helm_front_build *p) {
+    helm_tuning_refresh();
+    if (!p || p->nz < 1 || p->nx < 1 || p->dof < 1 || p->nf < 1 || p->nf > ND_NF_MAX || p->mode < 0 || p->mode > 2 || !p->image) return HELM_ERR_ARG;
+    const int nf = p->nf;
+    if (p->mode == 0 && (nf != 1 || p->skip22)) return HELM_ERR_ARG;
+    NdPlanDev pd;
+    nd_build_plan(pd.plan, p->nz, p->nx, p->leaf, p->dof);
+    const NdPlan &P = pd.plan;
+    if (p->group < 0 || p->group >= (int)P.groups.size()) return HELM_ERR_ARG;
+    const NdGroup &g = P.groups[p->group];
+    const int nmax = g.smax + g.mmax;
+    if (!((size_t)nmax * sizeof(int2) <= 64 * 1024 && nd_asm_packs(P.dof, P.nz, P.nx, nmax))) return HELM_ERR_UNSUPPORTED;
+    const long long N = (long long)P.nz * P.nx, plane_elems = P.dof > 2 ? 27 * N * P.dof : (P.dof == 2 ? 36 * N : 9 * N);
+    if (p->planes_len != plane_elems) return HELM_ERR_ARG;
+    for (int k = 0; k < nf; ++k) if (!p->planes[k]) return HELM_ERR_ARG;
+    if (p->mode == 2 && (p->front < 0 || p->front >= g.cnt || p->kf < 0 || p->kf >= nf)) return HELM_ERR_ARG;
+    const long long nimg = p->mode == 2 ? 1 : (long long)g.cnt * nf;
+    if (p->image_len != nimg * nmax * nmax) return HELM_ERR_ARG;
+    const long long fs = (long long)g.mmax * nmax, s1 = (long long)g.smax * nmax;
+    const size_t na = (size_t)(2 * P.fregion * nf), nfac = (size_t)(P.fac_elems * nf), nlu = (size_t)std::max<long long>(1, s1);
+    std::vector<unsigned long long> hA(2 * na, BF_SENTINEL), hF(2 * nfac, BF_SENTINEL), hL(2 * nlu, BF_SENTINEL);
+    for (int j = 0; j < g.cnt; ++j)
+        for (int c = 0; c < 2; ++c) {
+            const int kid = P.nodes[g.first + j].kid[c];
+            if (kid < 0) continue;
+            const NdDev &cn = P.nodes[kid];
+            const long long slot = (long long)cn.mmax * (cn.smax + cn.mmax);
+            for (int k = 0; k < nf; ++k)
+                for (long long i = 0; i < slot; ++i)
+                    for (int part = 0; part < 2; ++part) {
+                        const double v = bf_seed_value(p->seed, p->freq_id[k], cn.foff + i, part);
+                        memcpy(&hA[2 * ((long long)nf * cn.foff + (long long)k * slot + i) + part], &v, 8);
+                    }
+        }
+    const std::vector<unsigned long long> hA0 = hA;
+    if (hipSetDevice(p->device) != hipSuccess) return HELM_ERR_DEVICE;
+    cplx *dA = nullptr, *dF = nullptr, *dL = nullptr, *dP[ND_NF_MAX] = {nullptr, nullptr, nullptr, nullptr};
+    bool ok = hipMalloc((void **)&pd.d_nodes, P.nodes.size() * sizeof(NdDev)) == hipSuccess && hipMalloc((void **)&pd.d_asm, (size_t)P.total_rows * sizeof(int2)) == hipSuccess &&
+              hipMalloc((void **)&dA, na * 16) == hipSuccess && hipMalloc((void **)&dF, std::max<size_t>(nfac, 1) * 16) == hipSuccess && hipMalloc((void **)&dL, nlu * 16) == hipSuccess;
+    for (int k = 0; ok && k < nf; ++k) ok = hipMalloc((void **)&dP[k], (size_t)plane_elems * 16) == hipSuccess;
+    int rc = HELM_OK;
+    if (ok) {
+        hipMemcpy(pd.d_nodes, P.nodes.data(), P.nodes.size() * sizeof(NdDev), hipMemcpyHostToDevice);
+        hipMemcpy(dA, hA.data(), na * 16, hipMemcpyHostToDevice);
+        hipMemcpy(dF, hF.data(), nfac * 16, hipMemcpyHostToDevice);
+        hipMemcpy(dL, hL.data(), nlu * 16, hipMemcpyHostToDevice);
+        for (int k = 0; k < nf; ++k) hipMemcpy(dP[k], p->planes[k], (size_t)plane_elems * 16, hipMemcpyHostToDevice);
+        nd_launch_build_asm(nullptr, P, pd.d_nodes, pd.d_asm);
+        if (p->mode == 0) rc = launch_build_scatter(nullptr, nullptr, &pd, g, dA, dF, dP[0]);
+        else if (p->mode == 1) {
+            NdPlanesSet ps; for (int k = 0; k < ND_NF_MAX; ++k) ps.p[k] = dP[k < nf ? k : 0];
+            const int chunk = 65535 / nf;
+            for (int j0 = 0; j0 < g.cnt; j0 += chunk) launch_build_front(nullptr, &pd, g, j0, std::min(chunk, g.cnt - j0), dA, dF, ps, p->skip22 ? 1 : 0, nf);
+        } else {
+            NdDev n = P.nodes[g.first + p->front];
+            n.finv_off = 0; n.f12_off = g.smax;
+            launch_build_front_one(nullptr, &pd, n, dA, dL, dP[p->kf], nf, p->kf);
+        }
+        if (hipDeviceSynchronize() != hipSuccess || hipGetLastError() != hipSuccess) rc = HELM_ERR_DEVICE;
+        hipMemcpy(hA.data(), dA, na * 16, hipMemcpyDeviceToHost);
+        hipMemcpy(hF.data(), dF, nfac * 16, hipMemcpyDeviceToHost);
+        hipMemcpy(hL.data(), dL, nlu * 16, hipMemcpyDeviceToHost);
+    } else rc = HELM_ERR_DEVICE;
+    hipFree(pd.d_nodes); hipFree(pd.d_asm); pd.d_nodes = nullptr; pd.d_asm = nullptr;
+    hipFree(dA); hipFree(dF); hipFree(dL);
+    for (int k = 0; k < nf; ++k) hipFree(dP[k]);
+    if (rc) return rc;
+    unsigned long long *img = (unsigned long long *)p->image;
+    long long a_lo, a_hi, f_lo, f_hi;
+    if (p->mode == 2) {
+        const NdDev &n = P.nodes[g.first + p->front];
+        a_lo = (long long)nf * n.foff + (long long)p->kf * fs; a_hi = a_lo + fs; f_lo = f_hi = 0;
+        for (long long r = 0; r < nmax; ++r)
+            memcpy(img + 2 * r * nmax, r < g.smax ? &hL[2 * r * nmax] : &hA[2 * (a_lo + (r - g.smax) * nmax)], (size_t)nmax * 16);
+    } else {
+        a_lo = (long long)nf * g.foff; a_hi = a_lo + (long long)nf * g.cnt * fs; f_lo = (long long)nf * g.finv; f_hi = f_lo + (long long)nf * g.cnt * s1;
+        for (long long b = 0; b < nimg; ++b)
+            for (long long r = 0; r < nmax; ++r)
+                memcpy(img + 2 * (b * nmax + r) * nmax, r < g.smax ? &hF[2 * (f_lo + b * s1 + r * nmax)] : &hA[2 * (a_lo + b * fs + (r - g.smax) * nmax)], (size_t)nmax * 16);
+    }
+    long long stray = 0;
+    for (long long i = 0; i < (long long)na; ++i) if (i < a_lo || i >= a_hi) stray += (hA[2 * i] != hA0[2 * i]) + (hA[2 * i + 1] != hA0[2 * i + 1]);
+    for (long long i = 0; i < (long long)nfac; ++i) if (i < f_lo || i >= f_hi) stray += (hF[2 * i] != BF_SENTINEL) + (hF[2 * i + 1] != BF_SENTINEL);
+    if (p->mode != 2) for (size_t i = 0; i < 2 * nlu; ++i) stray += hL[i] != BF_SENTINEL;
+    p->stray = stray;
+    p->sentinel = BF_SENTINEL;
+    return HELM_OK;
+}
diff --git a/zephyr_amd/csrc/nd_internal.hpp b/zephyr_amd/csrc/nd_internal.hpp
--- a/zephyr_amd/csrc/nd_internal.hpp
+++ b/zephyr_amd/csrc/nd_internal.hpp
@@ -163,6 +163,7 @@
     }
 };
 
+void nd_launch_build_asm(hipStream_t st, const NdPlan &P, const NdDev *d_nodes, int2 *d_asm);
 struct GemmChoice { int tile = 0, kslab = 8, xr = 0, ksplit = 0, kc = 0; };
 int gemm(helm_op *op, int M, int Nn, int K, cplx alpha, const cplx *A, int lda, long long sa, const cplx *B, int ldb, long long sb,
          cplx beta, cplx *C, int ldc, long long sc, int batch, const GemmRows *rows = nullptr, GemmChoice *made = nullptr);
diff --git a/zephyr_amd/csrc/nd_plan.hip b/zephyr_amd/csrc/nd_plan.hip
--- a/zephyr_amd/csrc/nd_plan.hip
+++ b/zephyr_amd/csrc/nd_plan.hip
@@ -153,11 +153,33 @@
     }
 }
 
+__global__ __launch_bounds__(256) void k_nd_build_asm(const NdDev *nodes, int first, int2 *tab, int nz, int nx) {
+    const NdDev n = nodes[first + blockIdx.y];
+    const int nmax = n.smax + n.mmax;
+    const bool h0 = n.kid[0] >= 0, h1 = n.kid[1] >= 0;
+    NdDev c0 = NdDev(), c1 = NdDev();
+    if (h0) c0 = nodes[n.kid[0]];
+    if (h1) c1 = nodes[n.kid[1]];
+    for (int row = blockIdx.x * blockDim.x + threadIdx.x; row < nmax; row += gridDim.x * blockDim.x)
+        tab[n.roff + row] = nd_asm_entry(n, h0 ? &c0 : nullptr, h1 ? &c1 : nullptr, nz, nx, row);
+}
+
+}
+void nd_launch_build_asm(hipStream_t st, const NdPlan &P, const NdDev *d_nodes, int2 *d_asm) {
+    for (size_t gi = 0; gi < P.groups.size(); ++gi) {
+        const NdGroup &g = P.groups[gi];
+        const int nmax = g.smax + g.mmax;
+        for (int j0 = 0; j0 < g.cnt; j0 += 65535) {
+            const int nb = std::min(65535, g.cnt - j0);
+            HELM_LAUNCH(k_nd_build_asm, dim3((nmax + 255) / 256, nb), dim3(256), 0, st, d_nodes, g.first + j0, d_asm, P.nz, P.nx);
+        }
+    }
 }
 
 NdPlanDev::~NdPlanDev() {
     if (d_nodes) helm_pool_free(device, d_nodes, plan.nodes.size() * sizeof(NdDev));
     if (d_tab) helm_pool_free(device, d_tab, (size_t)plan.total_rows * sizeof(int4));
+    if (d_asm) helm_pool_free(device, d_asm, (size_t)plan.total_rows * sizeof(int2));
     if (d_cellnode) helm_pool_free(device, d_cellnode, (size_t)plan.nz * plan.nx * sizeof(int));
 }
 
@@ -193,7 +215,8 @@
     if (2 * P.vregion >= (1LL << 31) || P.total_rows >= (1LL << 31)) HELM_FAIL(op, HELM_ERR_UNSUPPORTED, "direct solver: grid too large for 32-bit row indices");
     pd->d_nodes = (NdDev *)helm_pool_alloc(op->device, P.nodes.size() * sizeof(NdDev));
     pd->d_tab = (int4 *)helm_pool_alloc(op->device, (size_t)P.total_rows * sizeof(int4));
-    if (!pd->d_nodes || !pd->d_tab) HELM_FAIL(op, HELM_ERR_DEVICE, "direct solver: allocation of the plan tables failed");
+    pd->d_asm = (int2 *)helm_pool_alloc(op->device, (size_t)P.total_rows * sizeof(int2));
+    if (!pd->d_nodes || !pd->d_tab || !pd->d_asm) HELM_FAIL(op, HELM_ERR_DEVICE, "direct solver: allocation of the plan tables failed");
     HIP_TRY(op, hipMemcpyAsync(pd->d_nodes, P.nodes.data(), P.nodes.size() * sizeof(NdDev), hipMemcpyHostToDevice, op->stream));
     for (size_t gi = 0; gi < P.groups.size(); ++gi) {
         const NdGroup &g = P.groups[gi];
@@ -203,6 +226,7 @@
             HELM_LAUNCH(k_nd_build_tab, dim3((nmax + 255) / 256, nb), dim3(256), 0, op->stream, pd->d_nodes, g.first + j0, pd->d_tab, P.nz, P.nx);
         }
     }
+    nd_launch_build_asm(op->stream, P, pd->d_nodes, pd->d_asm);
     if (dof == 1) {
         pd->d_cellnode = (int *)helm_pool_alloc(op->device, (size_t)pnz * pnx * sizeof(int));
         if (pd->d_cellnode) {
@@ -252,6 +276,53 @@
     return nn;
 }
 
+extern "C" int helm_debug_plan_nodes(int nz, int nx, int leaf, int dof, long long *out, int cap) {
+    helm_tuning_refresh();
+    if (nz < 1 || nx < 1 || dof < 1) return HELM_ERR_ARG;
+    NdPlan P;
+    nd_build_plan(P, nz, nx, leaf, dof);
+    const int nn = (int)P.nodes.size();
+    if (!out) return nn;
+    std::vector<int> group(nn, -1);
+    for (size_t gi = 0; gi < P.groups.size(); ++gi) for (int j = 0; j < P.groups[gi].cnt; ++j) group[P.groups[gi].first + j] = (int)gi;
+    for (int i = 0; i < nn && i < cap; ++i) {
+        const NdDev &n = P.nodes[i];
+        long long *o = out + 16 * i;
+        o[0] = n.z0; o[1] = n.z1; o[2] = n.x0; o[3] = n.x1; o[4] = n.cut; o[5] = n.pos; o[6] = n.s; o[7] = n.m;
+        o[8] = n.kid[0]; o[9] = n.kid[1]; o[10] = n.smax; o[11] = n.mmax; o[12] = n.roff; o[13] = group[i]; o[14] = P.groups[group[i]].level; o[15] = P.groups[group[i]].leaf ? 1 : 0;
+    }
+    return nn;
+}
+
+extern "C" long long helm_debug_asm_table(int device, int nz, int nx, int leaf, int dof, int *out, long long cap_rows) {
+    helm_tuning_refresh();
+    if (nz < 1 || nx < 1 || dof < 1) return HELM_ERR_ARG;
+    NdPlan P;
+    nd_build_plan(P, nz, nx, leaf, dof);
+    if (!out) return P.total_rows;
+    if (cap_rows < P.total_rows) return HELM_ERR_ARG;
+    if (device < 0) {
+        for (const NdDev &n : P.nodes)
+            for (int r = 0; r < n.smax + n.mmax; ++r) {
+                const int2 e = nd_asm_entry(n, n.kid[0] >= 0 ? &P.nodes[n.kid[0]] : nullptr, n.kid[1] >= 0 ? &P.nodes[n.kid[1]] : nullptr, nz, nx, r);
+                out[2 * (n.roff + r)] = e.x; out[2 * (n.roff + r) + 1] = e.y;
+            }
+        return P.total_rows;
+    }
+    if (hipSetDevice(device) != hipSuccess) return HELM_ERR_DEVICE;
+    NdDev *d_nodes = nullptr; int2 *d_asm = nullptr;
+    if (hipMalloc((void **)&d_nodes, P.nodes.size() * sizeof(NdDev)) != hipSuccess || hipMalloc((void **)&d_asm, (size_t)P.total_rows * sizeof(int2)) != hipSuccess) {
+        hipFree(d_nodes); return HELM_ERR_DEVICE;
+    }
+    hipMemcpy(d_nodes, P.nodes.data(), P.nodes.size() * sizeof(NdDev), hipMemcpyHostToDevice);
+    hipMemset(d_asm, 0x5A, (size_t)P.total_rows * sizeof(int2));
+    nd_launch_build_asm(nullptr, P, d_nodes, d_asm);
+    const hipError_t e = hipDeviceSynchronize();
+    hipMemcpy(out, d_asm, (size_t)P.total_rows * sizeof(int2), hipMemcpyDeviceToHost);
+    hipFree(d_nodes); hipFree(d_asm);
+    return e == hipSuccess ? P.total_rows : (long long)HELM_ERR_DEVICE;
+}
+
 extern "C" int helm_direct_plan_front(int nz, int nx, int leaf, int node, long long *cells, int cap) {
     helm_tuning_refresh();
     NdPlan P;
```

New measurement: 14640. 8.0% lower.
